# OliBomby/CM3P

Measured on AMD Instinct MI355X. Metric: contrastive training steps/sec (global beatmap-metadata pairs/sec), higher is better.
Workload: dtype bf16; 1 GPU; c2: default CM3P config, beatmap seq=4096, metadata seq=256, batch 32/GPU; global_batch=32, beatmap_seq=4096, metadata_seq=256, parallelism=dp1, weights=random init (reference init rules), fp32 master / bf16 GEMM operands

## Files before the change

### cm3p_amd/_lib.py

```python
from __future__ import annotations

import ctypes
import os
from ctypes import c_float, c_int, c_int64, c_uint64, c_void_p

import torch

F32, BF16 = 0, 1
ADD_A_BF16 = 16
POOL_PACKED = 2
GEMM_F32_TILED = 2
EPI_BF16, EPI_F32, EPI_F32_RESID, EPI_F32_BIAS, EPI_BF16_RESID = 0, 1, 2, 5, 7
ABI_VERSION = 20

_HERE = os.path.dirname(os.path.abspath(__file__))
LIB_PATH = os.environ.get("CM3P_HIP_LIB") or os.path.join(_HERE, "csrc", "libcm3p_hip.so")

_P, _I, _L, _F, _U64 = c_void_p, c_int, c_int64, c_float, c_uint64
_RETURNS_INT64 = {"cm3p_attn_bwd_fused_workspace_bytes", "cm3p_token_order_workspace_ints"}

SIGNATURES = {
    "cm3p_abi_version": [],
    "cm3p_layernorm_fwd": [_P, _I, _P, _P, _P, _P, _P, _L, _I, _F, _P],
    "cm3p_layernorm_bwd_blocks": [_L],
    "cm3p_layernorm_bwd": [_P, _I, _P, _I, _P, _P, _P, _P, _I, _P, _P, _P, _P, _L, _I, _P],
    "cm3p_embed_ln_fwd": [_P, _P, _I, _P, _P, _I, _P, _P, _P, _P, _P, _L, _I, _F, _L, _P],
    "cm3p_embed_ln_bwd": [_P, _I, _P, _P, _I, _P, _P, _I, _P, _P, _P, _P, _P, _P, _P, _L, _I, _L, _L, _P],
    "cm3p_embed_ln_bwd_sorted_chunk": [],
    "cm3p_embed_ln_bwd_sorted": [_P, _I, _P, _P, _P, _P, _I, _P, _P, _I, _P, _P, _P, _P, _P, _P, _P, _P, _P, _L, _I, _L, _L, _P],
    "cm3p_token_order_workspace_ints": [_L, _L],
    "cm3p_token_order": [_P, _L, _L, _P, _P, _P, _P],
    "cm3p_audio_slots": [_P, _L, _L, _P, _P, _P],
    "cm3p_gemm_bf16": [_P, _P, _P, _P, _L, _L, _L, _L, _L, _L, _I, _I, _I, _I, _P, _P],
    "cm3p_qkv_gemm_rope": [_P, _P, _P, _L, _L, _L, _P, _P, _I, _I, _I, _F, _P],
    "cm3p_gemm_wgrad_splits": [_L, _L, _L],
    "cm3p_gemm_route": [_L, _L, _L, _L, _L, _I, _I, _I, _I, _I, _I],
    "cm3p_gemm8p_set_grid": [_I],
    "cm3p_gemm8p_get_grid": [],
    "cm3p_build_ablation_flags": [],
    "cm3p_debug_set_dma_audit": [_P],
    "cm3p_cast_f32_bf16": [_P, _P, _L, _P],
    "cm3p_cast_f32_bf16_t": [_P, _P, _P, _L, _L, _P],
    "cm3p_cast_f32_bf16_t_multi": [_P, _I, _L, _P],
    "cm3p_add_f32": [_P, _P, _I, _P, _P, _L, _P],
    "cm3p_rope_table": [_P, _L, _P, _I, _P, _P, _P],
    "cm3p_rope_apply": [_P, _P, _P, _I, _I, _I, _L, _I, _P],
    "cm3p_attn_fwd": [_P, _P, _P, _P, _I, _I, _I, _I, _F, _I, _P],
    "cm3p_attn_fwd_impl": [_I, _I, _I, _I],
    "cm3p_attn_probs": [_P, _P, _P, _P, _I, _I, _I, _I, _F, _I, _P],
    "cm3p_attn_generic_supported": [_I],
    "cm3p_attn_fwd_generic": [_P, _P, _P, _P, _I, _I, _I, _I, _I, _F, _P],
    "cm3p_attn_bwd_generic": [_P, _P, _P, _P, _P, _P, _P, _I, _I, _I, _I, _I, _F, _P],
    "cm3p_attn_fwd_generic_dropout": [_P, _P, _P, _P, _I, _I, _I, _I, _I, _F, _I, _I, _U64, _P],
    "cm3p_attn_bwd_generic_dropout": [_P, _P, _P, _P, _P, _P, _P, _I, _I, _I, _I, _I, _F, _I, _I, _U64, _P],
    "cm3p_rope_apply_generic": [_P, _P, _P, _I, _I, _I, _I, _L, _I, _P],
    "cm3p_attn_bwd": [_P, _P, _P, _P, _P, _P, _P, _I, _I, _I, _I, _F, _P, _P, _L, _I, _I, _P],
    "cm3p_geglu_fwd": [_P, _P, _L, _I, _P],
    "cm3p_gemm_geglu": [_P, _P, _P, _L, _L, _L, _P],
    "cm3p_geglu_bwd": [_P, _P, _P, _L, _I, _P],
    "cm3p_dropout_f32": [_P, _P, _P, _P, _L, _I, _I, _P, _I, _I, _I, _I, _U64, _P],
    "cm3p_attn_fwd_dropout": [_P, _P, _P, _P, _I, _I, _I, _I, _F, _I, _I, _I, _U64, _P],
    "cm3p_attn_bwd_dropout": [_P, _P, _P, _P, _P, _P, _P, _I, _I, _I, _I, _F, _P, _P, _L, _I, _I, _I, _I, _U64, _P],
    "cm3p_attn_fwd_dropout_varlen": [_P, _P, _P, _P, _I, _I, _L, _I, _I, _F, _I, _I, _I, _U64, _P],
    "cm3p_attn_bwd_dropout_varlen": [_P, _P, _P, _P, _P, _P, _P, _I, _I, _L, _I, _I, _F, _P, _P, _I, _I, _I, _I, _U64, _P],
    "cm3p_geglu_fwd_dropout": [_P, _P, _L, _I, _I, _P, _I, _I, _I, _U64, _P],
    "cm3p_geglu_bwd_dropout": [_P, _P, _P, _L, _I, _I, _P, _I, _I, _I, _U64, _P],
    "cm3p_dropout_keep": [_P, _I, _I, _I, _I, _I, _I, _U64, _P],
    "cm3p_philox4x32_10_host": [_P, _P, _P, _L],
    "cm3p_gelu_fwd": [_P, _P, _L, _P],
    "cm3p_gelu_bwd": [_P, _P, _P, _L, _P],
    "cm3p_im2col_k3": [_P, _I, _P, _I, _I, _I, _I, _I, _P],
    "cm3p_col2im_k3": [_P, _P, _I, _I, _I, _I, _I, _P],
    "cm3p_bias_gelu_fwd": [_P, _P, _P, _P, _L, _I, _P],
    "cm3p_bias_gelu_bwd_blocks": [_L],
    "cm3p_bias_gelu_bwd": [_P, _I, _P, _P, _P, _P, _P, _L, _I, _P],
    "cm3p_pool_chunks": [_I],
    "cm3p_pool_fwd": [_P, _I, _P, _P, _P, _P, _I, _I, _I, _I, _P],
    "cm3p_pool_bwd": [_P, _P, _P, _P, _I, _I, _I, _I, _I, _P],
    "cm3p_gemm_f32": [_P, _P, _P, _I, _I, _I, _L, _L, _L, _L, _L, _F, _I, _P],
    "cm3p_l2norm_fwd": [_P, _P, _P, _I, _I, _P],
    "cm3p_l2norm_bwd": [_P, _P, _P, _P, _I, _I, _P],
    "cm3p_cross_entropy": [_P, _I, _I, _L, _L, _P, _P, _F, _P, _P, _P],
    "cm3p_cross_entropy_masked": [_P, _L, _I, _L, _P, _L, _F, _P, _P, _P, _P],
    "cm3p_inv_valid_count": [_P, _L, _L, _P, _P],
    "cm3p_ce_masked_stats": [_P, _L, _I, _L, _P, _L, _P, _P, _P],
    "cm3p_ce_masked_dlogits_blocks": [_L],
    "cm3p_ce_masked_dlogits_bf16": [_P, _L, _I, _L, _P, _L, _P, _P, _P, _P, _P, _P, _P],
    "cm3p_add_bias_f32": [_P, _P, _L, _I, _P],
    "cm3p_colsum_blocks": [_L],
    "cm3p_colsum_f32": [_P, _P, _P, _L, _I, _P],
    "cm3p_first_zero_index": [_P, _I, _I, _P, _P],
    "cm3p_scale_exp": [_P, _P, _P, _L, _P],
    "cm3p_scale_by": [_P, _P, _P, _L, _P],
    "cm3p_dot_f32": [_P, _P, _P, _L, _P],
    "cm3p_sum_f32": [_P, _P, _L, _F, _I, _P],
# ... 158 lines not shown
```

### cm3p_amd/csrc/common.h

```cpp
#pragma once
#include <hip/hip_runtime.h>
#include <stdint.h>

#include <atomic>
#include <initializer_list>
#include <mutex>
#include <type_traits>

#include "../../include/cm3p_hip.h"

typedef __attribute__((ext_vector_type(8))) __bf16 bf16x8;
typedef __attribute__((ext_vector_type(4))) __bf16 bf16x4;
typedef __attribute__((ext_vector_type(2))) __bf16 bf16x2;
typedef __attribute__((ext_vector_type(4))) float f32x4;
typedef __attribute__((ext_vector_type(8))) float f32x8;
typedef __attribute__((ext_vector_type(16))) float f32x16;

#define CM3P_WAVE 64
#define CM3P_EPI_BF16_ROPE 3
#define CM3P_EPI_BF16_AXPBY 4
#define CM3P_EPI_BF16_GEGLU 6

struct BatchArgs {
    int64_t a_stride = 0, b_stride = 0, c_stride = 0, r_stride = 0;
    const uint16_t* Rb = nullptr;
    float alpha = 1.f, beta = 0.f;
};

#ifndef CM3P_NT
#define CM3P_NT 7
#endif
typedef __attribute__((ext_vector_type(4))) uint32_t cm3p_u32x4;
typedef __attribute__((ext_vector_type(2))) uint32_t cm3p_u32x2;
template <bool NT>
__device__ __forceinline__ void gstore16(void* p, cm3p_u32x4 v) {
    if constexpr (NT) __builtin_nontemporal_store(v, static_cast<cm3p_u32x4*>(p));
    else *static_cast<cm3p_u32x4*>(p) = v;
}
template <bool NT>
__device__ __forceinline__ void gstore16(void* p, uint4 v) { gstore16<NT>(p, cm3p_u32x4{v.x, v.y, v.z, v.w}); }
template <bool NT>
__device__ __forceinline__ void gstore16f(void* p, __attribute__((ext_vector_type(4))) float v) {
    gstore16<NT>(p, __builtin_bit_cast(cm3p_u32x4, v));
}
template <bool NT>
__device__ __forceinline__ void gstore8(void* p, uint2 v) {
    if constexpr (NT) __builtin_nontemporal_store(cm3p_u32x2{v.x, v.y}, static_cast<cm3p_u32x2*>(p));
    else *static_cast<uint2*>(p) = v;
}
template <bool NT>
__device__ __forceinline__ uint4 gload16(const void* p) {
    if constexpr (NT) {
        const cm3p_u32x4 v = __builtin_nontemporal_load(static_cast<const cm3p_u32x4*>(p));
        return uint4{v[0], v[1], v[2], v[3]};
    } else {
        return *static_cast<const uint4*>(p);
    }
}

template <bool NT>
__device__ __forceinline__ uint2 gload8(const void* p) {
    if constexpr (NT) {
        const cm3p_u32x2 v = __builtin_nontemporal_load(static_cast<const cm3p_u32x2*>(p));
        return uint2{v[0], v[1]};
    } else {
        return *static_cast<const uint2*>(p);
    }
}
template <bool NT>
__device__ __forceinline__ __attribute__((ext_vector_type(4))) float gload16f(const void* p) {
    typedef __attribute__((ext_vector_type(4))) float f4;
    if constexpr (NT) return __builtin_nontemporal_load(static_cast<const f4*>(p));
    else return *static_cast<const f4*>(p);
}

#ifndef CM3P_DMA_AUDIT
#define CM3P_DMA_AUDIT 0
#endif
enum { CM3P_AUD_A = 0, CM3P_AUD_B = 1, CM3P_AUD_T0 = 2, CM3P_AUD_T1 = 3, CM3P_AUD_S0 = 4, CM3P_AUD_S1 = 5, CM3P_AUD_SLOTS = 8 };
#if CM3P_DMA_AUDIT
static __device__ unsigned long long* cm3p_audit_buf = nullptr;
static inline int cm3p_audit_set_local(void* buf) {
    return hipMemcpyToSymbol(HIP_SYMBOL(cm3p_audit_buf), &buf, sizeof(buf)) == hipSuccess ? CM3P_OK : CM3P_ERR_LAUNCH;
}
__device__ __forceinline__ void cm3p_audit(int id, const void* first_byte, int bytes) {
    unsigned long long* buf = cm3p_audit_buf;
    if (!buf) return;
    unsigned long long lo = (unsigned long long)(uintptr_t)first_byte, hi = lo + (unsigned long long)bytes - 1ull;
#pragma unroll
    for (int o = 32; o > 0; o >>= 1) {
        const unsigned long long l2 = __shfl_xor(lo, o, 64), h2 = __shfl_xor(hi, o, 64);
        lo = l2 < lo ? l2 : lo;
        hi = h2 > hi ? h2 : hi;
    }
    if ((threadIdx.x & 63) == 0) {
        atomicMin(buf + 2 * id, lo);
        atomicMax(buf + 2 * id + 1, hi);
    }
}
#define CM3P_AUDIT(id, addr, bytes) cm3p_audit((id), (addr), (bytes))
#else
#define CM3P_AUDIT(id, addr, bytes) ((void)0)
#endif

#define CM3P_LAUNCH_CHECK()                                         \
    do {                                                            \
        hipError_t e__ = hipGetLastError();                         \
        if (e__ != hipSuccess) return CM3P_ERR_LAUNCH;              \
    } while (0)
// ... 15 lines not shown
    if (cu[d] == 0) {
        hipDeviceProp_t prop;
        cu[d] = (hipGetDeviceProperties(&prop, d) == hipSuccess && prop.multiProcessorCount > 0) ? prop.multiProcessorCount : 256;
    }
    return cu[d];
}
struct Cm3pDevOnce {
    std::atomic<unsigned char> done[kCm3pMaxDevices] = {};
    std::mutex mu;
    template <class F>
    int run(F&& body) {
        int d = 0;
        const bool tracked = hipGetDevice(&d) == hipSuccess && d >= 0 && d < kCm3pMaxDevices;
        if (tracked && done[d].load(std::memory_order_acquire)) return CM3P_OK;
        std::lock_guard<std::mutex> g(mu);
        if (tracked && done[d].load(std::memory_order_relaxed)) return CM3P_OK;
        const int rc = body();
        if (rc == CM3P_OK && tracked) done[d].store(1, std::memory_order_release);
        return rc;
    }
};

static inline int cm3p_set_max_lds(std::initializer_list<const void*> kernels, int bytes) {
    for (const void* k : kernels)
        if (hipFuncSetAttribute(k, hipFuncAttributeMaxDynamicSharedMemorySize, bytes) != hipSuccess) return CM3P_ERR_LAUNCH;
    return CM3P_OK;
}

static inline bool cm3p_aligned16(const void* p) { return (reinterpret_cast<uintptr_t>(p) & 15u) == 0; }

__device__ __forceinline__ float bf16_bits_to_f32(uint16_t b) { return __builtin_bit_cast(float, (uint32_t)b << 16); }
__device__ __forceinline__ uint16_t f32_to_bf16_bits(float f) { return __builtin_bit_cast(uint16_t, (__bf16)f); }

typedef __attribute__((ext_vector_type(2))) float f32x2;
__device__ __forceinline__ f32x2 gelu_q_poly(f32x2 t) {
    f32x2 q = t * 0.24651730060577393f + (-1.1861149072647095f);
    q = q * t + 2.147474527359009f;
    q = q * t + (-1.6377531290054321f);
    q = q * t + 0.40232157707214355f;
    q = q * t + (-0.2687568664550781f);
    q = q * t + 0.1396300494670868f;
    q = q * t + 0.5397006273269653f;
    q = q * t + 1.4427292346954346f;
    q = q * t + (-1.8257482051849365f);
    return q;
}
__device__ __forceinline__ f32x2 gelu_t(f32x2 x) {
    const f32x2 ax = {__builtin_fabsf(x.x), __builtin_fabsf(x.y)};
    const f32x2 w = ax * 0.35355339059327373f + 1.0f;
    return f32x2{__builtin_amdgcn_rcpf(w.x), __builtin_amdgcn_rcpf(w.y)};
}
__device__ __forceinline__ void gelu_cdf_pdf2(f32x2 x, f32x2& cdf, f32x2& pdf) {
    const f32x2 t = gelu_t(x);
    const f32x2 q = gelu_q_poly(t);
    const f32x2 u = x * x * (-0.72134752044448170f);
    const f32x2 eu = {__builtin_amdgcn_exp2f(u.x), __builtin_amdgcn_exp2f(u.y)};
    const f32x2 eq = {__builtin_amdgcn_exp2f(q.x), __builtin_amdgcn_exp2f(q.y)};
    const f32x2 h = t * eu * eq * 0.5f;
    cdf.x = x.x < 0.f ? h.x : 1.0f - h.x;
    cdf.y = x.y < 0.f ? h.y : 1.0f - h.y;
    pdf = eu * 0.39894228040143267794f;
}
__device__ __forceinline__ f32x2 gelu_erf2(f32x2 x) {
    const f32x2 t = gelu_t(x);
    const f32x2 e = x * x * (-0.72134752044448170f) + gelu_q_poly(t);
    const f32x2 h = t * f32x2{__builtin_amdgcn_exp2f(e.x), __builtin_amdgcn_exp2f(e.y)} * 0.5f;
    const f32x2 cdf = {x.x < 0.f ? h.x : 1.0f - h.x, x.y < 0.f ? h.y : 1.0f - h.y};
    return x * cdf;
}
__device__ __forceinline__ f32x2 gelu_erf_grad2(f32x2 x) {
    f32x2 cdf, pdf;
    gelu_cdf_pdf2(x, cdf, pdf);
    return x * pdf + cdf;
}

__device__ __forceinline__ uint32_t pack_bf16x2(float lo, float hi) {
    bf16x2 v = {(__bf16)lo, (__bf16)hi};
    return __builtin_bit_cast(uint32_t, v);
}
__device__ __forceinline__ float bf16lo(uint32_t w) { return __builtin_bit_cast(float, w << 16); }
__device__ __forceinline__ float bf16hi(uint32_t w) { return __builtin_bit_cast(float, w & 0xffff0000u); }
__device__ __forceinline__ uint32_t add_bf16x2(uint32_t a, uint32_t b) { return pack_bf16x2(bf16lo(a) + bf16lo(b), bf16hi(a) + bf16hi(b)); }

struct RopeArgs {
    const float* cos;
    const float* sin;
    int S;
    int per_batch;
    int ncols;
    int q_cols = 0;
    float q_scale = 1.f;
};

enum { CM3P_GEMM_128 = 0, CM3P_GEMM_256 = 1, CM3P_GEMM_RING = 2 };
struct GemmRoute {
    int kernel;
    bool rebal;
    int splits;
    int64_t kchunk;
};
struct GemmCall {
    const void* A;
    const void* B;
    void* C;
    const float* R;
    int64_t M, N, K, lda, ldb, ldc;
    int a_kc, b_kc, epi;
    int64_t c_split_stride = 0;
    RopeArgs rope = RopeArgs{};
    BatchArgs bt = BatchArgs{};
    int batch = 0;
};
template <class F>
int cm3p_with_flag(bool v, F&& f) {
    return v ? f(std::true_type{}) : f(std::false_type{});
}
template <class F>
int cm3p_with_layout(bool a_kc, bool b_kc, F&& f) {
    return cm3p_with_flag(a_kc, [&](auto ak) { return cm3p_with_flag(b_kc, [&](auto bk) { return f(ak, bk); }); });
}
template <class F>
int cm3p_with_epilogue(int epi, F&& f) {
    switch (epi) {
        case CM3P_EPI_BF16: return f(std::integral_constant<int, CM3P_EPI_BF16>{});
        case CM3P_EPI_F32: return f(std::integral_constant<int, CM3P_EPI_F32>{});
        case CM3P_EPI_F32_RESID: return f(std::integral_constant<int, CM3P_EPI_F32_RESID>{});
        case CM3P_EPI_BF16_ROPE: return f(std::integral_constant<int, CM3P_EPI_BF16_ROPE>{});
        case CM3P_EPI_BF16_AXPBY: return f(std::integral_constant<int, CM3P_EPI_BF16_AXPBY>{});
        case CM3P_EPI_F32_BIAS: return f(std::integral_constant<int, CM3P_EPI_F32_BIAS>{});
        case CM3P_EPI_BF16_GEGLU: return f(std::integral_constant<int, CM3P_EPI_BF16_GEGLU>{});
        case CM3P_EPI_BF16_RESID: return f(std::integral_constant<int, CM3P_EPI_BF16_RESID>{});
        default: return CM3P_ERR_INTERNAL;
    }
}
constexpr bool cm3p_gemm_pair_exists(bool a_kc, bool b_kc, int epi) {
    return (epi != CM3P_EPI_BF16_ROPE && epi != CM3P_EPI_F32_BIAS && epi != CM3P_EPI_BF16_GEGLU) || (a_kc && b_kc);
}

template <bool INVERSE>
__device__ __forceinline__ void rope_rotate4(f32x4& a, f32x4& b, const float* cos_row, const float* sin_row, int d) {
    const f32x4 cs = *reinterpret_cast<const f32x4*>(cos_row + d);
    const f32x4 sn = *reinterpret_cast<const f32x4*>(sin_row + d);
    const f32x4 a0 = a, b0 = b;
    if constexpr (!INVERSE) {
        a = a0 * cs - b0 * sn;
        b = b0 * cs + a0 * sn;
    } else {
        a = a0 * cs + b0 * sn;
        b = b0 * cs - a0 * sn;
    }
}

__device__ __forceinline__ float wave_sum(float v) {
#pragma unroll
    for (int o = 32; o > 0; o >>= 1) v += __shfl_xor(v, o, 64);
    return v;
}
__device__ __forceinline__ float wave_max(float v) {
#pragma unroll
    for (int o = 32; o > 0; o >>= 1) v = fmaxf(v, __shfl_xor(v, o, 64));
    return v;
}

__device__ __forceinline__ bf16x4 lds_read_tr16(const void* p) {
    return __builtin_amdgcn_ds_read_tr16_b64_v4bf16((__attribute__((address_space(3))) bf16x4*)(p));
}

__device__ __forceinline__ bf16x8 cat_bf16x4(bf16x4 a, bf16x4 b) {
    return __builtin_shufflevector(a, b, 0, 1, 2, 3, 4, 5, 6, 7);
}
```

### cm3p_amd/csrc/elementwise.hip

```cpp
#include "common.h"
#include "dropout_rng.h"

namespace {

inline int ew_grid(int64_t items, int per_block = 256) {
    int64_t blocks = (items + per_block - 1) / per_block;
    if (blocks > 2048) blocks = 2048;
    if (blocks < 1) blocks = 1;
    return (int)blocks;
}

__device__ __forceinline__ void unpack8(const uint4 w, float (&f)[8]) {
    f[0] = bf16lo(w.x); f[1] = bf16hi(w.x); f[2] = bf16lo(w.y); f[3] = bf16hi(w.y);
    f[4] = bf16lo(w.z); f[5] = bf16hi(w.z); f[6] = bf16lo(w.w); f[7] = bf16hi(w.w);
}
__device__ __forceinline__ uint4 pack8(const float (&f)[8]) {
    return uint4{pack_bf16x2(f[0], f[1]), pack_bf16x2(f[2], f[3]), pack_bf16x2(f[4], f[5]), pack_bf16x2(f[6], f[7])};
}

__global__ __launch_bounds__(256) void cast_f32_bf16_kernel(const float* __restrict__ x, uint16_t* __restrict__ y, int64_t n4) {
    for (int64_t i = (int64_t)blockIdx.x * 256 + threadIdx.x; i < n4; i += (int64_t)gridDim.x * 256) {
        const f32x4 v = reinterpret_cast<const f32x4*>(x)[i];
        reinterpret_cast<uint2*>(y)[i] = uint2{pack_bf16x2(v.x, v.y), pack_bf16x2(v.z, v.w)};
    }
}

__global__ __launch_bounds__(256) void cast_f32_bf16_t_kernel(const float* __restrict__ x, uint16_t* __restrict__ y, uint16_t* __restrict__ yt,
                                                              int rows, int cols, int tiles_c) {
    __shared__ uint16_t tile[64][66];
    const int r0 = (blockIdx.x / tiles_c) * 64, c0 = (blockIdx.x % tiles_c) * 64;
    const int tid = threadIdx.x;
#pragma unroll
    for (int it = 0; it < 4; ++it) {
        const int r = it * 16 + (tid >> 4), c = (tid & 15) * 4;
        if (r0 + r < rows && c0 + c < cols) {
            const f32x4 v = *reinterpret_cast<const f32x4*>(x + (int64_t)(r0 + r) * cols + c0 + c);
            const uint32_t lo = pack_bf16x2(v.x, v.y), hi = pack_bf16x2(v.z, v.w);
            *reinterpret_cast<uint2*>(y + (int64_t)(r0 + r) * cols + c0 + c) = uint2{lo, hi};
            tile[r][c] = (uint16_t)lo;
            tile[r][c + 1] = (uint16_t)(lo >> 16);
            tile[r][c + 2] = (uint16_t)hi;
            tile[r][c + 3] = (uint16_t)(hi >> 16);
        }
    }
    __syncthreads();
#pragma unroll
    for (int it = 0; it < 2; ++it) {
        const int c = it * 32 + (tid >> 3), r = (tid & 7) * 8;
        if (c0 + c < cols && r0 + r < rows) {
            uint32_t w[4];
#pragma unroll
            for (int k = 0; k < 4; ++k) w[k] = (uint32_t)tile[r + 2 * k][c] | ((uint32_t)tile[r + 2 * k + 1][c] << 16);
            *reinterpret_cast<uint4*>(yt + (int64_t)(c0 + c) * rows + r0 + r) = uint4{w[0], w[1], w[2], w[3]};
        }
    }
}

__global__ __launch_bounds__(256) void cast_f32_bf16_t_multi_kernel(const int64_t* __restrict__ table, int n) {
    __shared__ uint16_t tile[64][66];
    int lo = 0, hi = n - 1;
    while (lo < hi) {
        const int mid = (lo + hi + 1) >> 1;
        if (table[6 * mid + 5] <= (int64_t)blockIdx.x) lo = mid;
        else hi = mid - 1;
    }
    const float* x = reinterpret_cast<const float*>(table[6 * lo]);
    uint16_t* y = reinterpret_cast<uint16_t*>(table[6 * lo + 1]);
    uint16_t* yt = reinterpret_cast<uint16_t*>(table[6 * lo + 2]);
    const int rows = (int)table[6 * lo + 3], cols = (int)table[6 * lo + 4];
    const int blk = (int)((int64_t)blockIdx.x - table[6 * lo + 5]);
    const int tiles_c = (cols + 63) / 64;
    const int r0 = (blk / tiles_c) * 64, c0 = (blk % tiles_c) * 64;
    const int tid = threadIdx.x;
#pragma unroll
    for (int it = 0; it < 4; ++it) {
        const int r = it * 16 + (tid >> 4), c = (tid & 15) * 4;
        if (r0 + r < rows && c0 + c < cols) {
            const f32x4 v = *reinterpret_cast<const f32x4*>(x + (int64_t)(r0 + r) * cols + c0 + c);
            const uint32_t lo2 = pack_bf16x2(v.x, v.y), hi2 = pack_bf16x2(v.z, v.w);
            *reinterpret_cast<uint2*>(y + (int64_t)(r0 + r) * cols + c0 + c) = uint2{lo2, hi2};
            tile[r][c] = (uint16_t)lo2;
            tile[r][c + 1] = (uint16_t)(lo2 >> 16);
            tile[r][c + 2] = (uint16_t)hi2;
            tile[r][c + 3] = (uint16_t)(hi2 >> 16);
        }
    }
    __syncthreads();
#pragma unroll
    for (int it = 0; it < 2; ++it) {
        const int c = it * 32 + (tid >> 3), r = (tid & 7) * 8;
        if (c0 + c < cols && r0 + r < rows) {
            uint32_t w[4];
#pragma unroll
            for (int k = 0; k < 4; ++k) w[k] = (uint32_t)tile[r + 2 * k][c] | ((uint32_t)tile[r + 2 * k + 1][c] << 16);
            *reinterpret_cast<uint4*>(yt + (int64_t)(c0 + c) * rows + r0 + r) = uint4{w[0], w[1], w[2], w[3]};
        }
    }
}

template <bool B_BF16>
__global__ __launch_bounds__(256) void add_f32_kernel(const float* __restrict__ a, const void* __restrict__ b, float* y32,
                                                      uint16_t* __restrict__ y16, int64_t n4) {
    for (int64_t i = (int64_t)blockIdx.x * 256 + threadIdx.x; i < n4; i += (int64_t)gridDim.x * 256) {
        f32x4 v = reinterpret_cast<const f32x4*>(a)[i];
        if constexpr (B_BF16) {
            const uint2 w = reinterpret_cast<const uint2*>(b)[i];
            v += f32x4{bf16lo(w.x), bf16hi(w.x), bf16lo(w.y), bf16hi(w.y)};
        } else {
            v += reinterpret_cast<const f32x4*>(b)[i];
        }
        if (y32) reinterpret_cast<f32x4*>(y32)[i] = v;
        if (y16) reinterpret_cast<uint2*>(y16)[i] = uint2{pack_bf16x2(v.x, v.y), pack_bf16x2(v.z, v.w)};
    }
}

template <bool B_BF16>
__global__ __launch_bounds__(256) void add_bf16_kernel(const uint16_t* a, const void* __restrict__ b, uint16_t* y, int64_t n4) {
    for (int64_t i = (int64_t)blockIdx.x * 256 + threadIdx.x; i < n4; i += (int64_t)gridDim.x * 256) {
        const uint2 wa = reinterpret_cast<const uint2*>(a)[i];
        f32x4 v = f32x4{bf16lo(wa.x), bf16hi(wa.x), bf16lo(wa.y), bf16hi(wa.y)};
        if constexpr (B_BF16) {
            const uint2 w = reinterpret_cast<const uint2*>(b)[i];
            v += f32x4{bf16lo(w.x), bf16hi(w.x), bf16lo(w.y), bf16hi(w.y)};
        } else {
            v += reinterpret_cast<const f32x4*>(b)[i];
        }
        reinterpret_cast<uint2*>(y)[i] = uint2{pack_bf16x2(v.x, v.y), pack_bf16x2(v.z, v.w)};
    }
}

__global__ __launch_bounds__(256) void rope_table_kernel(const int64_t* __restrict__ pos, const float* __restrict__ inv_freq,
                                                         float* __restrict__ cos_out, float* __restrict__ sin_out, int64_t n,
                                                         int half) {
    for (int64_t i = (int64_t)blockIdx.x * 256 + threadIdx.x; i < n * half; i += (int64_t)gridDim.x * 256) {
        const int64_t p = i / half;
        const int j = (int)(i % half);
        const float ang = (float)pos[p] * inv_freq[j];
        cos_out[i] = cosf(ang);
        sin_out[i] = sinf(ang);
    }
}

template <bool INVERSE>
__global__ __launch_bounds__(256) void rope_apply_kernel(uint16_t* __restrict__ qkv, const float* __restrict__ cos_tab,
                                                         const float* __restrict__ sin_tab, int64_t T, int S, int nh,
                                                         int64_t pos_batch_stride) {
    const int64_t per_tok = (int64_t)2 * nh * 4;
    const int64_t total = T * per_tok;
    for (int64_t i = (int64_t)blockIdx.x * 256 + threadIdx.x; i < total; i += (int64_t)gridDim.x * 256) {
        const int64_t t = i / per_tok;
        const int r = (int)(i % per_tok);
        const int part = r / (nh * 4);
        const int h = (r / 4) % nh;
        const int c = r & 3;
        const int64_t b = t / S, s = t % S;
        const int64_t prow = (pos_batch_stride ? b * pos_batch_stride : 0) + s;
        uint16_t* base = qkv + (t * 3 + part) * (int64_t)nh * 64 + h * 64 + c * 8;
        float x1[8], x2[8], cs[8], sn[8];
        unpack8(*reinterpret_cast<const uint4*>(base), x1);
        unpack8(*reinterpret_cast<const uint4*>(base + 32), x2);
        const f32x4* cp = reinterpret_cast<const f32x4*>(cos_tab + prow * 32 + c * 8);
        const f32x4* sp = reinterpret_cast<const f32x4*>(sin_tab + prow * 32 + c * 8);
        const f32x4 c0 = cp[0], c1 = cp[1], s0 = sp[0], s1 = sp[1];
// ... 3 lines not shown
#pragma unroll
        for (int j = 0; j < 8; ++j) {
            if constexpr (!INVERSE) {
                y1[j] = x1[j] * cs[j] - x2[j] * sn[j];
                y2[j] = x2[j] * cs[j] + x1[j] * sn[j];
            } else {
                y1[j] = x1[j] * cs[j] + x2[j] * sn[j];
                y2[j] = x2[j] * cs[j] - x1[j] * sn[j];
            }
        }
        *reinterpret_cast<uint4*>(base) = pack8(y1);
        *reinterpret_cast<uint4*>(base + 32) = pack8(y2);
    }
}

#ifndef CM3P_GEGLU_X2
#define CM3P_GEGLU_X2 3
#endif
template <int NI>
struct GegluWalk {
    int64_t dq, t0;
    int dr, c0, c8;
    __device__ __forceinline__ GegluWalk(int I) {
        c8 = I / 8;
        const int64_t stride = (int64_t)gridDim.x * 256 * NI, first = ((int64_t)blockIdx.x * 4 + (threadIdx.x >> 6)) * (64 * NI) + (threadIdx.x & 63);
        dq = stride / c8;
        dr = (int)(stride % c8);
        t0 = first / c8;
        c0 = (int)(first % c8);
    }
    __device__ __forceinline__ bool next(int64_t T, int64_t (&tt)[NI], int (&cc)[NI], bool (&ok)[NI]) {
        if (t0 >= T) return false;
        if (c0 >= c8) {
            c0 -= c8;
            if (++t0 >= T) return false;
        }
        tt[0] = t0, cc[0] = c0, ok[0] = true;
#pragma unroll
        for (int k = 1; k < NI; ++k) {
            tt[k] = tt[k - 1];
            cc[k] = cc[k - 1] + 64;
            while (cc[k] >= c8) {
                cc[k] -= c8;
                ++tt[k];
            }
            ok[k] = tt[k] < T;
            if (!ok[k]) tt[k] = t0, cc[k] = c0;
        }
        t0 += dq;
        c0 += dr;
        return true;
    }
};

__global__ __launch_bounds__(256) void geglu_fwd_kernel(const uint16_t* __restrict__ h, uint16_t* __restrict__ g, int64_t T, int I) {
    constexpr int NI = CM3P_GEGLU_X2 + 1;
    GegluWalk<NI> walk(I);
    int64_t tt[NI];
    int cc[NI];
    bool ok[NI];
    while (walk.next(T, tt, cc, ok)) {
        uint4 ha[NI], hb[NI];
#pragma unroll
        for (int k = 0; k < NI; ++k) {
            ha[k] = gload16<(CM3P_NT & 128) != 0>(h + tt[k] * 2 * I + cc[k] * 8);
            hb[k] = gload16<(CM3P_NT & 128) != 0>(h + tt[k] * 2 * I + I + cc[k] * 8);
        }
#pragma unroll
        for (int k = 0; k < NI; ++k) {
            float a[8], b[8], y[8];
            unpack8(ha[k], a);
            unpack8(hb[k], b);
#pragma unroll
            for (int j = 0; j < 8; j += 2) {
                const f32x2 gl = gelu_erf2(f32x2{a[j], a[j + 1]});
                y[j] = gl.x * b[j];
                y[j + 1] = gl.y * b[j + 1];
            }
            if (ok[k]) gstore16<(CM3P_NT & 16) != 0>(g + tt[k] * I + cc[k] * 8, pack8(y));
        }
    }
}

__device__ __forceinline__ void geglu_bwd_item_f(const uint4 ha, const uint4 hb, const float (&d)[8], uint4& oa, uint4& ob) {
    float a[8], b[8], da[8], db[8];
    unpack8(ha, a);
    unpack8(hb, b);
#pragma unroll
    for (int j = 0; j < 8; j += 2) {
        const f32x2 av = {a[j], a[j + 1]};
        f32x2 cdf, pdf;
        gelu_cdf_pdf2(av, cdf, pdf);
        const f32x2 gr = av * pdf + cdf, gl = av * cdf;
        da[j] = d[j] * b[j] * gr.x;
        da[j + 1] = d[j + 1] * b[j + 1] * gr.y;
        db[j] = d[j] * gl.x;
        db[j + 1] = d[j + 1] * gl.y;
    }
    oa = pack8(da);
    ob = pack8(db);
}

__device__ __forceinline__ void geglu_bwd_item(const uint4 ha, const uint4 hb, const uint4 hd, uint4& oa, uint4& ob) {
    float d[8];
    unpack8(hd, d);
    geglu_bwd_item_f(ha, hb, d, oa, ob);
}

__global__ __launch_bounds__(256) void geglu_bwd_kernel(const uint16_t* __restrict__ dg, const uint16_t* __restrict__ h,
                                                        uint16_t* __restrict__ dh, int64_t T, int I) {
    constexpr int NI = CM3P_GEGLU_X2 + 1;
    GegluWalk<NI> walk(I);
    int64_t tt[NI];
    int cc[NI];
    bool ok[NI];
    while (walk.next(T, tt, cc, ok)) {
        uint4 ha[NI], hb[NI], hd[NI];
#pragma unroll
        for (int k = 0; k < NI; ++k) {
            ha[k] = gload16<(CM3P_NT & 128) != 0>(h + tt[k] * 2 * I + cc[k] * 8);
            hb[k] = gload16<(CM3P_NT & 128) != 0>(h + tt[k] * 2 * I + I + cc[k] * 8);
            hd[k] = gload16<(CM3P_NT & 128) != 0>(dg + tt[k] * I + cc[k] * 8);
        }
#pragma unroll
        for (int k = 0; k < NI; ++k) {
            uint4 oa, ob;
            geglu_bwd_item(ha[k], hb[k], hd[k], oa, ob);
            if (ok[k]) {
                gstore16<(CM3P_NT & 16) != 0>(dh + tt[k] * 2 * I + cc[k] * 8, oa);
                gstore16<(CM3P_NT & 16) != 0>(dh + tt[k] * 2 * I + I + cc[k] * 8, ob);
            }
        }
    }
}

struct DropArgs {
    uint64_t seed;
    uint32_t c3, thr;
    float scale;
    int S, nseq;
    const int* cu;
};

__device__ __forceinline__ uint32_t drop_keep8(const DropArgs& d, int64_t t, uint32_t f8) {
    uint32_t b, s;
    cm3p_drop::row_to_seq(t, d.S, d.cu, d.nseq, b, s);
    return cm3p_drop::keep8(d.seed, f8, s, b, d.c3, d.thr);
}

__global__ __launch_bounds__(256) void dropout_f32_kernel(const float* x, const float* resid, float* y32, uint16_t* __restrict__ y16, int64_t rows,
                                                          int H, DropArgs d) {
    const int h8 = H / 8;
    const int64_t n = rows * h8;
    for (int64_t i = (int64_t)blockIdx.x * 256 + threadIdx.x; i < n; i += (int64_t)gridDim.x * 256) {
        const int64_t t = i / h8;
        const uint32_t m = drop_keep8(d, t, (uint32_t)(i - t * h8));
        f32x4 v0 = reinterpret_cast<const f32x4*>(x)[2 * i], v1 = reinterpret_cast<const f32x4*>(x)[2 * i + 1];
#pragma unroll
        for (int j = 0; j < 4; ++j) {
            v0[j] = (m >> j) & 1u ? v0[j] * d.scale : 0.f;
            v1[j] = (m >> (4 + j)) & 1u ? v1[j] * d.scale : 0.f;
        }
        if (resid) {
            v0 += reinterpret_cast<const f32x4*>(resid)[2 * i];
            v1 += reinterpret_cast<const f32x4*>(resid)[2 * i + 1];
        }
        if (y32) {
            reinterpret_cast<f32x4*>(y32)[2 * i] = v0;
            reinterpret_cast<f32x4*>(y32)[2 * i + 1] = v1;
        }
        if (y16)
            reinterpret_cast<uint4*>(y16)[i] =
                uint4{pack_bf16x2(v0.x, v0.y), pack_bf16x2(v0.z, v0.w), pack_bf16x2(v1.x, v1.y), pack_bf16x2(v1.z, v1.w)};
    }
}

__global__ __launch_bounds__(256) void geglu_drop_fwd_kernel(const uint16_t* __restrict__ h, uint16_t* __restrict__ g, int64_t T, int I,
                                                             DropArgs d) {
    const int i8 = I / 8;
    const int64_t n = T * i8;
    for (int64_t i = (int64_t)blockIdx.x * 256 + threadIdx.x; i < n; i += (int64_t)gridDim.x * 256) {
        const int64_t t = i / i8;
        const int c = (int)(i - t * i8);
        const uint32_t m = drop_keep8(d, t, (uint32_t)c);
        float a[8], b[8], y[8];
// ... 505 lines not shown
```

### cm3p_amd/csrc/gemm.hip

```cpp
#include <stdlib.h>

#include "common.h"

namespace {

constexpr int BM = 128, BN = 128, BK = 64;
constexpr int kStageBytes = BM * BK * 2;

__device__ __forceinline__ int kc_off(int r, int c) { return r * 128 + ((c ^ (r & 7)) << 4); }
__device__ __forceinline__ int ks_off(int k, int idx) {
    const int f = (k & 3) | (((k >> 3) & 1) << 2);
    return k * 256 + ((((idx >> 4) ^ f) & 7) << 5) + ((idx & 15) << 1);
}

template <bool KC>
struct TileLoader {
    const uint16_t* ptr[4];
    bool row_ok[4];
    int koff[4];
    int lds[4];
    int64_t kstep;

    __device__ __forceinline__ void init(const uint16_t* base, int64_t ld, int64_t idx0, int64_t extent, int64_t kbeg, int tid) {
#pragma unroll
// ... 90 lines not shown
        const char* sb = sa + kStageBytes;
        const bool more = kt + 1 < nk;
        if (more) {
            la.load(ra, kbeg + (int64_t)(kt + 1) * BK, kend);
            lb.load(rb, kbeg + (int64_t)(kt + 1) * BK, kend);
        }
#pragma unroll
        for (int kk = 0; kk < 2; ++kk) {
            bf16x8 fa[4], fb[4];
#pragma unroll
            for (int i = 0; i < 4; ++i) fa[i] = load_frag<A_KC>(sa, wm * 64 + i * 16, kk, lane);
#pragma unroll
            for (int j = 0; j < 4; ++j) fb[j] = load_frag<B_KC>(sb, wn * 64 + j * 16, kk, lane);
#pragma unroll
            for (int i = 0; i < 4; ++i)
#pragma unroll
                for (int j = 0; j < 4; ++j)
                    acc[i][j] = __builtin_amdgcn_mfma_f32_16x16x32_bf16(fb[j], fa[i], acc[i][j], 0, 0, 0);
        }
        if (more) {
            char* na = smem + ((kt + 1) & 1) * 2 * kStageBytes;
            la.store(na, ra);
            lb.store(na + kStageBytes, rb);
        }
        __syncthreads();
    }

#pragma unroll
    for (int i = 0; i < 4; ++i) {
        const int64_t m = m0 + wm * 64 + i * 16 + (lane & 15);
        if (m >= M) continue;
        if constexpr (EPI == CM3P_EPI_BF16_ROPE) {
            if (n0 + wn * 64 < rope.ncols) {
                const int64_t prow = rope.per_batch ? m : m % rope.S;
#pragma unroll
                for (int j = 0; j < 2; ++j)
                    rope_rotate4<false>(acc[i][j], acc[i][j + 2], rope.cos + prow * 32, rope.sin + prow * 32, j * 16 + 4 * (lane >> 4));
                if (n0 + wn * 64 < rope.q_cols) {
#pragma unroll
                    for (int j = 0; j < 4; ++j) acc[i][j] *= rope.q_scale;
                }
            }
        }
#pragma unroll
        for (int j = 0; j < 4; ++j) {
            const int64_t n = n0 + wn * 64 + j * 16 + 4 * (lane >> 4);
            if (n >= N) continue;
            f32x4 v = acc[i][j];
            if constexpr (EPI == CM3P_EPI_BF16 || EPI == CM3P_EPI_BF16_ROPE) {
                uint16_t* C = static_cast<uint16_t*>(Cv);
                *reinterpret_cast<uint2*>(C + m * ldc + n) = uint2{pack_bf16x2(v.x, v.y), pack_bf16x2(v.z, v.w)};
            } else if constexpr (EPI == CM3P_EPI_BF16_RESID) {
                uint16_t* C = static_cast<uint16_t*>(Cv);
                const uint2 r = *reinterpret_cast<const uint2*>(reinterpret_cast<const uint16_t*>(R) + m * ldc + n);
                *reinterpret_cast<uint2*>(C + m * ldc + n) = uint2{add_bf16x2(pack_bf16x2(v.x, v.y), r.x), add_bf16x2(pack_bf16x2(v.z, v.w), r.y)};
            } else if constexpr (EPI == CM3P_EPI_BF16_AXPBY) {
                uint16_t* C = static_cast<uint16_t*>(Cv) + (int64_t)blockIdx.y * bt.c_stride;
                v *= bt.alpha;
                if (bt.Rb) {
                    const uint2 r = *reinterpret_cast<const uint2*>(bt.Rb + (int64_t)blockIdx.y * bt.r_stride + m * ldc + n);
                    v += bt.beta * f32x4{bf16lo(r.x), bf16hi(r.x), bf16lo(r.y), bf16hi(r.y)};
                }
                *reinterpret_cast<uint2*>(C + m * ldc + n) = uint2{pack_bf16x2(v.x, v.y), pack_bf16x2(v.z, v.w)};
            } else {
                float* C = static_cast<float*>(Cv) + (int64_t)blockIdx.z * c_split_stride;
                if constexpr (EPI == CM3P_EPI_F32_RESID) v += *reinterpret_cast<const f32x4*>(R + m * ldc + n);
                if constexpr (EPI == CM3P_EPI_F32_BIAS) v += *reinterpret_cast<const f32x4*>(R + n);
                *reinterpret_cast<f32x4*>(C + m * ldc + n) = v;
            }
        }
    }
}

__global__ __launch_bounds__(256) void splitk_reduce_kernel(const float* __restrict__ ws, float* __restrict__ out, int64_t n4,
                                                            int splits, int64_t stride4) {
    for (int64_t i = (int64_t)blockIdx.x * 256 + threadIdx.x; i < n4; i += (int64_t)gridDim.x * 256) {
        f32x4 s = reinterpret_cast<const f32x4*>(ws)[i];
        for (int z = 1; z < splits; ++z) s += reinterpret_cast<const f32x4*>(ws)[i + z * stride4];
        reinterpret_cast<f32x4*>(out)[i] = s;
    }
}

template <bool A_KC, bool B_KC, int EPI>
constexpr bool has_instance = cm3p_gemm_pair_exists(A_KC, B_KC, EPI) && EPI != CM3P_EPI_BF16_GEGLU;

int launch128(const GemmRoute& r, const GemmCall& g, hipStream_t s) {
    const int tiles_m = (int)((g.M + BM - 1) / BM), tiles_n = (int)((g.N + BN - 1) / BN);
    const dim3 grid(tiles_m * tiles_n, g.batch > 0 ? g.batch : 1, r.splits);
    const size_t lds = 4 * kStageBytes;
    const uint16_t* a = static_cast<const uint16_t*>(g.A);
    const uint16_t* b = static_cast<const uint16_t*>(g.B);
    return cm3p_with_layout(g.a_kc, g.b_kc, [&](auto ak, auto bk) {
        return cm3p_with_epilogue(g.epi, [&](auto e) {
            constexpr bool AK = decltype(ak)::value, BK = decltype(bk)::value;
            constexpr int E = decltype(e)::value;
            if constexpr (has_instance<AK, BK, E>) {
                gemm_bf16_kernel<AK, BK, E><<<grid, 256, lds, s>>>(a, b, g.C, g.R, g.M, g.N, g.K, g.lda, g.ldb, g.ldc, tiles_n, r.kchunk,
                                                                 g.c_split_stride, g.rope, g.bt);
                return CM3P_OK;
            } else {
                return CM3P_ERR_INTERNAL;
            }
        });
    });
}

}

int cm3p_gemm256_dispatch(const GemmRoute& r, const GemmCall& g, hipStream_t s);
int cm3p_gemm8p_dispatch(const GemmRoute& r, const GemmCall& g, hipStream_t s);

static inline int64_t tiles_of(int64_t M, int64_t N, int t) { return ((M + t - 1) / t) * ((N + t - 1) / t); }
constexpr int64_t kBigItems = 200, kBigBatchItems = 128;

static GemmRoute cm3p_gemm_route_of(int64_t M, int64_t N, int64_t K, int64_t lda, int64_t ldb, bool a_kc, bool b_kc, int epi,
                                    int split_k, int rope_cols, int batch) {
    GemmRoute r{CM3P_GEMM_128, false, 1, K};
    const bool batched = epi == CM3P_EPI_BF16_AXPBY;
    if (M <= 0 || N <= 0 || K <= 0 || split_k < 1 || epi < 0 || epi > CM3P_EPI_BF16_RESID || batched != (batch > 0) ||
        !cm3p_gemm_pair_exists(a_kc, b_kc, epi)) {
        r.kernel = CM3P_ERR_INVALID;
        return r;
    }
    const char* impl = getenv("CM3P_GEMM_IMPL");
    const bool no_ring = impl && impl[0] == '2', small_only = impl && impl[0] == '1';
    static const bool no_rebal = [] { const char* e = getenv("CM3P_G8P_REBAL"); return e && e[0] == '0'; }();
    if (split_k > 1) {
        const int64_t q = (K % 128 == 0) ? 128 : 64;
        r.kchunk = ((K + split_k - 1) / split_k + q - 1) / q * q;
        r.splits = (int)((K + r.kchunk - 1) / r.kchunk);
    }
    const int64_t items = tiles_of(M, N, 256) * (batched ? batch : r.splits);
    const bool ring_ok = M % 8 == 0 && N % 8 == 0 && lda * 16 < (int64_t(1) << 31) && ldb * 16 < (int64_t(1) << 31);
    bool big = K % 64 == 0 && r.kchunk % 64 == 0 && items >= (batched ? kBigBatchItems : kBigItems);
    if (epi == CM3P_EPI_BF16_GEGLU) {
        if (!(big && N % 64 == 0 && ring_ok)) r.kernel = CM3P_ERR_INVALID;
        else r.kernel = no_ring ? CM3P_GEMM_256 : CM3P_GEMM_RING;
    } else if (batched) {
        const bool filled = M * N * batch * 10 >= items * 65536 * 7;
        big = big && filled && (a_kc || !b_kc) && ring_ok && !no_ring;
        if (big) r.kernel = CM3P_GEMM_RING;
    } else {
        big = big && !small_only;
        if (epi == CM3P_EPI_BF16_ROPE) big = big && rope_cols % 256 == 0 && M < (int64_t(1) << 31);
        if (big) r.kernel = (ring_ok && !no_ring) ? CM3P_GEMM_RING : CM3P_GEMM_256;
    }
    if (r.kernel > CM3P_GEMM_128) {
        const int64_t last = K - (int64_t)(r.splits - 1) * r.kchunk;
        r.rebal = !no_rebal && (r.kchunk / 64) % 2 == 0 && (last / 64) % 2 == 0;
    }
    return r;
}

static int run_routed(const GemmRoute& r, const GemmCall& g, hipStream_t s) {
    int rc = CM3P_ERR_INVALID;
    if (r.kernel == CM3P_GEMM_RING) rc = cm3p_gemm8p_dispatch(r, g, s);
    else if (r.kernel == CM3P_GEMM_256) rc = cm3p_gemm256_dispatch(r, g, s);
    else if (r.kernel == CM3P_GEMM_128) rc = launch128(r, g, s);
    if (rc != CM3P_OK) return rc;
    CM3P_LAUNCH_CHECK();
    return CM3P_OK;
}

int cm3p_ablation_flags_attention();
int cm3p_ablation_flags_attention_bwd_fused();
int cm3p_ablation_flags_gemm256();
int cm3p_ablation_flags_gemm8p();
int cm3p_ablation_flags_attention_fwd();
#if CM3P_DMA_AUDIT
int cm3p_audit_set_attention_fwd(void*);
int cm3p_audit_set_gemm8p(void*);
int cm3p_audit_set_gemm256(void*);
int cm3p_audit_set_attention(void*);
int cm3p_audit_set_attention_bwd_fused(void*);
#endif

extern "C" {

int cm3p_build_ablation_flags(void) {
    return (cm3p_ablation_flags_attention() != 0) | (cm3p_ablation_flags_attention_bwd_fused() != 0) << 2 |
           (cm3p_ablation_flags_gemm256() != 0) << 3 | (cm3p_ablation_flags_gemm8p() != 0) << 4 | (CM3P_DMA_AUDIT != 0) << 5 |
           (cm3p_ablation_flags_attention_fwd() != 0) << 6;
}

int cm3p_debug_set_dma_audit(void* buf) {
#if CM3P_DMA_AUDIT
    int rc = cm3p_audit_set_gemm8p(buf);
    if (rc == CM3P_OK) rc = cm3p_audit_set_gemm256(buf);
    if (rc == CM3P_OK) rc = cm3p_audit_set_attention(buf);
    if (rc == CM3P_OK) rc = cm3p_audit_set_attention_bwd_fused(buf);
    if (rc == CM3P_OK) rc = cm3p_audit_set_attention_fwd(buf);
    return rc;
#else
    (void)buf;
    return CM3P_ERR_INVALID;
#endif
}

int cm3p_gemm_wgrad_splits(int64_t M, int64_t N, int64_t K) {
    const int64_t t256 = tiles_of(M, N, 256);
    if (K % 64 == 0 && K >= 8192) {
        int64_t s = 256 / t256;
        if (s > K / 2048) s = K / 2048;
        if (s < 1) s = 1;
        if (t256 * s >= kBigItems) return (int)s;
    }
    const int64_t t128 = tiles_of(M, N, 128);
    if (t128 >= 512 || K <= 1024) return 1;
    int64_t s = (1024 + t128 - 1) / t128;
    if (s > K / 512) s = K / 512;
    return (int)(s < 1 ? 1 : s);
}

int cm3p_gemm_route(int64_t M, int64_t N, int64_t K, int64_t lda, int64_t ldb, int a_kc, int b_kc, int epilogue, int split_k,
                    int rope_cols, int batch) {
    const GemmRoute r = cm3p_gemm_route_of(M, N, K, lda, ldb, a_kc != 0, b_kc != 0, epilogue, split_k, rope_cols, batch);
    return r.kernel < 0 ? CM3P_ERR_INVALID : (r.kernel | (r.rebal ? 4 : 0) | r.splits << 3);
}

int cm3p_qkv_gemm_rope(const void* x, const void* Wqkv, void* qkv, int64_t M, int64_t N, int64_t K, const float* cos_tab,
                       const float* sin_tab, int S, int per_batch, int rope_cols, float q_scale, void* stream) {
    CM3P_REQUIRE(x && Wqkv && qkv && cos_tab && sin_tab && M > 0 && N > 0 && K > 0 && S > 0);
    CM3P_REQUIRE(cm3p_aligned16(x) && cm3p_aligned16(Wqkv) && cm3p_aligned16(qkv) && cm3p_aligned16(cos_tab) && cm3p_aligned16(sin_tab));
    CM3P_REQUIRE(K % 8 == 0 && N % 64 == 0 && rope_cols % 64 == 0 && rope_cols >= 0 && rope_cols <= N);
    CM3P_REQUIRE(per_batch || M % S == 0);
    CM3P_REQUIRE(q_scale > 0.f && rope_cols % 2 == 0);
    const GemmRoute r = cm3p_gemm_route_of(M, N, K, K, K, true, true, CM3P_EPI_BF16_ROPE, 1, rope_cols, 0);
    CM3P_REQUIRE(r.kernel >= 0);
    GemmCall g{x, Wqkv, qkv, nullptr, M, N, K, K, K, N, 1, 1, CM3P_EPI_BF16_ROPE};
    g.rope = RopeArgs{cos_tab, sin_tab, S, per_batch, rope_cols, rope_cols / 2, q_scale};
    return run_routed(r, g, static_cast<hipStream_t>(stream));
}

int cm3p_gemm_bf16(const void* A, const void* B, void* C, const float* R, int64_t M, int64_t N, int64_t K, int64_t lda,
                   int64_t ldb, int64_t ldc, int a_kc, int b_kc, int epilogue, int split_k, float* workspace, void* stream) {
    CM3P_REQUIRE(A && B && C && M > 0 && N > 0 && K > 0);
    CM3P_REQUIRE((epilogue >= CM3P_EPI_BF16 && epilogue <= CM3P_EPI_F32_RESID) || epilogue == CM3P_EPI_F32_BIAS || epilogue == CM3P_EPI_BF16_RESID);
    CM3P_REQUIRE(cm3p_aligned16(A) && cm3p_aligned16(B) && cm3p_aligned16(C));
    CM3P_REQUIRE(lda % 8 == 0 && ldb % 8 == 0 && ldc % 4 == 0 && N % 4 == 0);
    CM3P_REQUIRE(a_kc ? (K % 8 == 0 && lda >= K) : (M % 8 == 0 && lda >= M));
    CM3P_REQUIRE(b_kc ? (K % 8 == 0 && ldb >= K) : (N % 8 == 0 && ldb >= N));
    CM3P_REQUIRE(ldc >= N);
    CM3P_REQUIRE((epilogue != CM3P_EPI_F32_RESID && epilogue != CM3P_EPI_F32_BIAS && epilogue != CM3P_EPI_BF16_RESID) || (R && cm3p_aligned16(R)));
    CM3P_REQUIRE(epilogue != CM3P_EPI_BF16_RESID || (N % 8 == 0 && ldc % 8 == 0));
    CM3P_REQUIRE(split_k >= 1 && (split_k == 1 || (epilogue == CM3P_EPI_F32 && workspace && cm3p_aligned16(workspace) && ldc == N)));
    const GemmRoute r = cm3p_gemm_route_of(M, N, K, lda, ldb, a_kc != 0, b_kc != 0, epilogue, split_k, 0, 0);
    CM3P_REQUIRE(r.kernel >= 0);
    hipStream_t s = static_cast<hipStream_t>(stream);
    GemmCall g{A, B, C, R, M, N, K, lda, ldb, ldc, a_kc != 0, b_kc != 0, epilogue};
    if (r.splits > 1) {
        g.C = workspace;
        g.c_split_stride = M * N;
    }
    const int rc = run_routed(r, g, s);
    if (rc != CM3P_OK) return rc;
    if (r.splits > 1) {
        const int64_t n4 = M * N / 4;
        int64_t blocks = (n4 + 255) / 256;
        if (blocks > 2048) blocks = 2048;
        splitk_reduce_kernel<<<(int)blocks, 256, 0, s>>>(workspace, static_cast<float*>(C), n4, r.splits, n4);
        CM3P_LAUNCH_CHECK();
    }
    return CM3P_OK;
}

int cm3p_gemm_geglu(const void* x, const void* w_interleaved, void* a, int64_t T, int64_t I, int64_t K, void* stream) {
    CM3P_REQUIRE(x && w_interleaved && a && T > 0 && I > 0 && K > 0);
    CM3P_REQUIRE(cm3p_aligned16(x) && cm3p_aligned16(w_interleaved) && cm3p_aligned16(a));
    GemmRoute r = cm3p_gemm_route_of(T, 2 * I, K, K, K, true, true, CM3P_EPI_BF16_GEGLU, 1, 0, 0);
    CM3P_REQUIRE(r.kernel >= 0);
    r.kernel = CM3P_GEMM_RING;
    const GemmCall g{x, w_interleaved, a, nullptr, T, 2 * I, K, K, K, I, 1, 1, CM3P_EPI_BF16_GEGLU};
    return run_routed(r, g, static_cast<hipStream_t>(stream));
}

int cm3p_gemm_bf16_batched(const void* A, const void* B, void* C, const void* R, int batch, int64_t M, int64_t N, int64_t K,
                           int64_t lda, int64_t ldb, int64_t ldc, int64_t stride_a, int64_t stride_b, int64_t stride_c,
                           int64_t stride_r, int a_kc, int b_kc, float alpha, float beta, void* stream) {
    CM3P_REQUIRE(A && B && C && batch > 0 && batch <= 65535 && M > 0 && N > 0 && K > 0);
    CM3P_REQUIRE(cm3p_aligned16(A) && cm3p_aligned16(B) && cm3p_aligned16(C) && (!R || cm3p_aligned16(R)));
    CM3P_REQUIRE(lda % 8 == 0 && ldb % 8 == 0 && ldc % 8 == 0 && N % 8 == 0 && ldc >= N);
    CM3P_REQUIRE(stride_a % 8 == 0 && stride_b % 8 == 0 && stride_c % 8 == 0 && stride_r % 8 == 0);
    CM3P_REQUIRE(a_kc ? (K % 8 == 0 && lda >= K) : (M % 8 == 0 && lda >= M));
    CM3P_REQUIRE(b_kc ? (K % 8 == 0 && ldb >= K) : (N % 8 == 0 && ldb >= N));
    const GemmRoute r = cm3p_gemm_route_of(M, N, K, lda, ldb, a_kc != 0, b_kc != 0, CM3P_EPI_BF16_AXPBY, 1, 0, batch);
    CM3P_REQUIRE(r.kernel >= 0);
    GemmCall g{A, B, C, nullptr, M, N, K, lda, ldb, ldc, a_kc != 0, b_kc != 0, CM3P_EPI_BF16_AXPBY};
    g.bt = BatchArgs{stride_a, stride_b, stride_c, stride_r, static_cast<const uint16_t*>(R), alpha, beta};
    g.batch = batch;
    return run_routed(r, g, static_cast<hipStream_t>(stream));
}

}
```

### cm3p_amd/csrc/gemm256.hip

```cpp
#include "common.h"

namespace {

constexpr int TM = 256, TN = 256, TK = 64;
#ifndef CM3P_G256_WN
#define CM3P_G256_WN 4
#endif
constexpr int kWN = CM3P_G256_WN;
constexpr int kThreads = 128 * kWN;
constexpr int kNJ = 16 / kWN;
constexpr int kWaveN = TN / kWN;
#ifndef CM3P_G256_ABL
#define CM3P_G256_ABL 0
#endif
constexpr int kPieces = 16 / kWN;
constexpr int kItems = 2048 / kThreads;
constexpr int kOperandBytes = TM * TK * 2;
constexpr int kStage = 2 * kOperandBytes;

__device__ __forceinline__ int kc_off(int r, int c) { return r * 128 + ((c ^ (r & 7)) << 4); }
__device__ __forceinline__ int ksf(int k) { return (k & 3) | (((k >> 3) & 1) << 2); }
__device__ __forceinline__ int ks_off(int k, int idx) { return k * 512 + (((idx >> 4) ^ ksf(k)) << 5) + ((idx & 15) << 1); }

__device__ __forceinline__ void glds16(const void* gsrc, char* lds_wave_base) {
// ... 250 lines not shown
                        if (m < M && n < N) {
                            uint4 x = *reinterpret_cast<const uint4*>(ebuf + r * kRow + ch * 16);
                            if constexpr (EPI == CM3P_EPI_BF16_RESID) {
                                const uint4 rb = *reinterpret_cast<const uint4*>(reinterpret_cast<const uint16_t*>(R) + m * ldc + n);
                                x = uint4{add_bf16x2(x.x, rb.x), add_bf16x2(x.y, rb.y), add_bf16x2(x.z, rb.z), add_bf16x2(x.w, rb.w)};
                            }
                            if constexpr (EPI == CM3P_EPI_BF16) {
                                if (n + 8 > N) {
                                    *reinterpret_cast<uint2*>(C + m * ldc + n) = uint2{x.x, x.y};
                                    continue;
                                }
                            }
                            *reinterpret_cast<uint4*>(C + m * ldc + n) = x;
                        }
                    }
                }
                lds_barrier();
            }
        } else {
            constexpr int kRow = TN * 4 + 16;
            float* C = static_cast<float*>(Cv) + (int64_t)z * c_split_stride;
            f32x4 rres[kItems];
            auto load_resid = [&](int pass) {
                if constexpr (EPI == CM3P_EPI_F32_RESID) {
#pragma unroll
                    for (int u = 0; u < kItems; ++u) {
                        const int id = tid + kThreads * u, r = id >> 6, ch = id & 63;
                        const int64_t m = m0 + pass * 32 + r, n = n0 + ch * 4;
                        rres[u] = (m < M && n < N) ? *reinterpret_cast<const f32x4*>(R + m * ldc + n) : f32x4{0.f, 0.f, 0.f, 0.f};
                    }
                }
                if constexpr (EPI == CM3P_EPI_F32_BIAS) {
                    if (pass == 0) {
#pragma unroll
                        for (int u = 0; u < kItems; ++u) {
                            const int64_t n = n0 + ((tid + kThreads * u) & 63) * 4;
                            rres[u] = n < N ? *reinterpret_cast<const f32x4*>(R + n) : f32x4{0.f, 0.f, 0.f, 0.f};
                        }
                    }
                }
            };
            load_resid(0);
#pragma unroll
            for (int pass = 0; pass < 8; ++pass) {
                if (wm == (pass >> 2)) {
#pragma unroll
                    for (int i2 = 0; i2 < 2; ++i2)
#pragma unroll
                        for (int j = 0; j < kNJ; ++j) {
                            const f32x4 a = acc[(pass & 3) * 2 + i2][j];
                            const int r = i2 * 16 + (lane & 15), cidx = wn * kWaveN + j * 16 + 4 * (lane >> 4);
                            *reinterpret_cast<f32x4*>(ebuf + r * kRow + cidx * 4) = a;
                        }
                }
                lds_barrier();
                f32x4 rcur[kItems];
#pragma unroll
                for (int u = 0; u < kItems; ++u) rcur[u] = rres[u];
                if (pass < 7) load_resid(pass + 1);
#pragma unroll
                for (int u = 0; u < kItems; ++u) {
                    const int id = tid + kThreads * u, r = id >> 6, ch = id & 63;
                    const int64_t m = m0 + pass * 32 + r, n = n0 + ch * 4;
                    if (m < M && n < N) {
                        f32x4 a = *reinterpret_cast<const f32x4*>(ebuf + r * kRow + ch * 16);
                        if constexpr (EPI == CM3P_EPI_F32_RESID || EPI == CM3P_EPI_F32_BIAS) a += rcur[u];
                        *reinterpret_cast<f32x4*>(C + m * ldc + n) = a;
                    }
                }
                lds_barrier();
            }
        }

        if (!has_next) break;
        v = vn;
        m0 = m0n;
        n0 = n0n;
        z = zn;
        nk = nkn;
    }
}

template <bool A_KC, bool B_KC, int EPI>
constexpr bool has_instance = cm3p_gemm_pair_exists(A_KC, B_KC, EPI) && EPI != CM3P_EPI_BF16_GEGLU && EPI != CM3P_EPI_BF16_AXPBY;

}

int cm3p_gemm256_dispatch(const GemmRoute& r, const GemmCall& g, hipStream_t s) {
    const int tiles_m = (int)((g.M + TM - 1) / TM), tiles_n = (int)((g.N + TN - 1) / TN);
    const int ntiles = tiles_m * tiles_n, total = ntiles * r.splits;
    const int num_cu = cm3p_num_cu();
    const dim3 grid(total < num_cu ? total : num_cu);
    const size_t lds = 2 * kStage;
    const uint16_t* a = static_cast<const uint16_t*>(g.A);
    const uint16_t* b = static_cast<const uint16_t*>(g.B);
    return cm3p_with_layout(g.a_kc, g.b_kc, [&](auto ak, auto bk) {
        return cm3p_with_epilogue(g.epi, [&](auto e) {
            constexpr bool AK = decltype(ak)::value, BK = decltype(bk)::value;
            constexpr int E = decltype(e)::value;
            if constexpr (has_instance<AK, BK, E>) {
                static Cm3pDevOnce once;
                const int rc_once = once.run([&] { return cm3p_set_max_lds({(const void*)gemm256_kernel<AK, BK, E>}, (int)lds); });
                if (rc_once != CM3P_OK) return rc_once;
                gemm256_kernel<AK, BK, E><<<grid, kThreads, lds, s>>>(a, b, g.C, g.R, g.M, g.N, g.K, g.lda, g.ldb, g.ldc, tiles_n, ntiles, total,
                                                                    r.kchunk, g.c_split_stride, g.rope);
                return CM3P_OK;
            } else {
                return CM3P_ERR_INTERNAL;
            }
        });
    });
}

int cm3p_ablation_flags_gemm256() { return (CM3P_G256_ABL) | ((CM3P_G256_WN != 4) << 8); }
#if CM3P_DMA_AUDIT
int cm3p_audit_set_gemm256(void* buf) { return cm3p_audit_set_local(buf); }
#endif
```

### cm3p_amd/csrc/gemm8p.hip

```cpp
#include <stdlib.h>

#include <type_traits>

#include "common.h"

#ifndef CM3P_G8P_ABL
#define CM3P_G8P_ABL 0
#endif
#ifndef CM3P_G8P_DELAY
#define CM3P_G8P_DELAY 10
#endif

namespace {

constexpr int kHalf = 16384;
constexpr int kRing = 8 * kHalf;
constexpr int kEpiWave = 4096;
constexpr int kLds8p = kRing + 8 * kEpiWave;
enum { kAL = 0, kAH = 1, kBL = 2, kBH = 3 };
__host__ __device__ constexpr int slot_off(int par, int kind) { return (par * 4 + kind) * kHalf; }

template <int IMM, int AUD = CM3P_AUD_A>
__device__ __forceinline__ void glds_s(uint32_t voff, const char* sbase, uint32_t ldsw) {
    CM3P_AUDIT(AUD, sbase + voff, 16);
// ... 306 lines not shown
                if constexpr (EPI == CM3P_EPI_BF16_RESID) {
                    const int r0 = lane >> 3, r1 = 8 + (lane >> 3), ch = lane & 7;
                    const bool col_ok = FULL || nw + ch * 8 < N;
                    res0 = (FULL || (col_ok && mw + i4 * 16 + r0 < M)) ? __builtin_bit_cast(u32x4, gload16<(CM3P_NT & 64) != 0>(Rb + (uint32_t)(i4 * 16 + r0) * ldcb + ch * 16))
                                                                       : u32x4{0u, 0u, 0u, 0u};
                    res1 = (FULL || (col_ok && mw + i4 * 16 + r1 < M)) ? __builtin_bit_cast(u32x4, gload16<(CM3P_NT & 64) != 0>(Rb + (uint32_t)(i4 * 16 + r1) * ldcb + ch * 16))
                                                                       : u32x4{0u, 0u, 0u, 0u};
                }
#pragma unroll
                for (int j4 = 0; j4 < 4; ++j4) {
                    const f32x4 a = acc[i4][j4];
                    const int row = lane & 15, s8 = (j4 * 4 + (lane >> 4)) ^ ((row & 7) << 1);
                    *reinterpret_cast<uint2*>(eb + row * 128 + s8 * 8) = uint2{pack_bf16x2(a.x, a.y), pack_bf16x2(a.z, a.w)};
                }
                G8P_LANE_XCHG_FENCE();
                if (rotate) {
                    const int row = lane >> 2, dc = lane & 3;
                    char* pa = eb + row * 128 + ((dc ^ (row & 7)) << 4);
                    char* pb = eb + row * 128 + (((dc + 4) ^ (row & 7)) << 4);
                    const u32x4 xa = *reinterpret_cast<const u32x4*>(pa);
                    const u32x4 xb = *reinterpret_cast<const u32x4*>(pb);
                    const f32x4 c0 = tc0, c1 = tc1, s0 = ts0, s1 = ts1;
                    if (i4 < 7) tab_load(i4 + 1, tc0, tc1, ts0, ts1);
                    {
                        const float cs[8] = {c0.x, c0.y, c0.z, c0.w, c1.x, c1.y, c1.z, c1.w};
                        const float sn[8] = {s0.x, s0.y, s0.z, s0.w, s1.x, s1.y, s1.z, s1.w};
                        u32x4 oa, ob;
#pragma unroll
                        for (int t = 0; t < 4; ++t) {
                            const float a0 = bf16lo(xa[t]), a1 = bf16hi(xa[t]), b0 = bf16lo(xb[t]), b1 = bf16hi(xb[t]);
                            oa[t] = pack_bf16x2(qs * (a0 * cs[2 * t] - b0 * sn[2 * t]), qs * (a1 * cs[2 * t + 1] - b1 * sn[2 * t + 1]));
                            ob[t] = pack_bf16x2(qs * (b0 * cs[2 * t] + a0 * sn[2 * t]), qs * (b1 * cs[2 * t + 1] + a1 * sn[2 * t + 1]));
                        }
                        *reinterpret_cast<u32x4*>(pa) = oa;
                        *reinterpret_cast<u32x4*>(pb) = ob;
                    }
                    G8P_LANE_XCHG_FENCE();
                }
                {
                    const int r0 = lane >> 3, r1 = 8 + (lane >> 3), ch = lane & 7;
                    u32x4 x0 = *reinterpret_cast<const u32x4*>(eb + r0 * 128 + ((ch ^ (r0 & 7)) << 4));
                    u32x4 x1 = *reinterpret_cast<const u32x4*>(eb + r1 * 128 + ((ch ^ (r1 & 7)) << 4));
                    G8P_LANE_XCHG_FENCE();
                    if constexpr (EPI == CM3P_EPI_BF16_RESID) {
#pragma unroll
                        for (int t = 0; t < 4; ++t) {
                            x0[t] = add_bf16x2(x0[t], res0[t]);
                            x1[t] = add_bf16x2(x1[t], res1[t]);
                        }
                    }
                    const bool col_ok = FULL || nw + ch * 8 < N;
                    if (FULL || (col_ok && mw + i4 * 16 + r0 < M)) G8P_GLOBAL(gstore16<(CM3P_NT & 1) != 0>(Cb + (uint32_t)(i4 * 16 + r0) * ldcb + ch * 16, x0));
                    if (FULL || (col_ok && mw + i4 * 16 + r1 < M)) G8P_GLOBAL(gstore16<(CM3P_NT & 1) != 0>(Cb + (uint32_t)(i4 * 16 + r1) * ldcb + ch * 16, x1));
                    if constexpr (CM3P_G8P_ABL & 1) asm volatile("" ::"v"(x0), "v"(x1));
                }
            }
        } else if constexpr (EPI == CM3P_EPI_BF16_GEGLU) {
            char* Cb = reinterpret_cast<char*>(static_cast<uint16_t*>(Cv) + mw * ldc + nw / 2);
            const uint32_t ldcb = (uint32_t)ldc * 2;
#pragma unroll
            for (int i4 = 0; i4 < 8; ++i4) {
                char* eb = ebuf + (i4 & 1) * 2048;
#pragma unroll
                for (int j4 = 0; j4 < 4; ++j4) {
                    const f32x4 a = acc[i4][j4];
                    const int row = lane & 15, s8 = (j4 * 4 + (lane >> 4)) ^ ((row & 7) << 1);
                    *reinterpret_cast<uint2*>(eb + row * 128 + s8 * 8) = uint2{pack_bf16x2(a.x, a.y), pack_bf16x2(a.z, a.w)};
                }
                G8P_LANE_XCHG_FENCE();
                const int row = lane >> 2, dc = lane & 3;
                const u32x4 xh = *reinterpret_cast<const u32x4*>(eb + row * 128 + ((dc ^ (row & 7)) << 4));
                const u32x4 xg = *reinterpret_cast<const u32x4*>(eb + row * 128 + (((dc + 4) ^ (row & 7)) << 4));
                G8P_LANE_XCHG_FENCE();
                u32x4 y;
#pragma unroll
                for (int t = 0; t < 4; ++t) {
                    const f32x2 gl = gelu_erf2(f32x2{bf16lo(xh[t]), bf16hi(xh[t])});
                    y[t] = pack_bf16x2(gl.x * bf16lo(xg[t]), gl.y * bf16hi(xg[t]));
                }
                if (FULL || (mw + i4 * 16 + row < M && nw + dc * 8 < N))
                    G8P_GLOBAL(gstore16<(CM3P_NT & 1) != 0>(Cb + (uint32_t)(i4 * 16 + row) * ldcb + dc * 16, y));
                if constexpr (CM3P_G8P_ABL & 1) asm volatile("" ::"v"(y));
            }
        } else if constexpr (EPI == CM3P_EPI_BF16_AXPBY) {
            char* Cb = reinterpret_cast<char*>(static_cast<uint16_t*>(Cv) + (int64_t)z * bt.c_stride + mw * ldc + nw);
            const char* Rb = reinterpret_cast<const char*>(bt.Rb + (int64_t)z * bt.r_stride + mw * ldc + nw);
            const uint32_t ldcb = (uint32_t)ldc * 2;
            const int lrow = lane >> 4, lch = lane & 15;
            const uint32_t loff = (uint32_t)lrow * ldcb + lch * 8;
            const bool col_ok = FULL || nw + lch * 4 < N;
#pragma unroll
            for (int i4 = 0; i4 < 8; ++i4) {
                uint2 r[4];
                if (bt.Rb) {
#pragma unroll
                    for (int u = 0; u < 4; ++u) {
                        const int row = i4 * 16 + u * 4;
                        r[u] = (FULL || (col_ok && mw + row + lrow < M)) ? *reinterpret_cast<const uint2*>(Rb + loff + (uint32_t)row * ldcb) : uint2{0u, 0u};
                    }
                }
#pragma unroll
                for (int j4 = 0; j4 < 4; ++j4) {
                    const int row = lane & 15, ch = j4 * 4 + (lane >> 4);
                    *reinterpret_cast<f32x4*>(ebuf + row * 256 + ((ch ^ row) << 4)) = acc[i4][j4];
                }
                G8P_LANE_XCHG_FENCE();
                f32x4 x[4];
#pragma unroll
                for (int u = 0; u < 4; ++u) {
                    const int row = u * 4 + lrow;
                    x[u] = *reinterpret_cast<const f32x4*>(ebuf + row * 256 + ((lch ^ row) << 4));
                }
                G8P_LANE_XCHG_FENCE();
#pragma unroll
                for (int u = 0; u < 4; ++u) {
                    f32x4 v = x[u];
                    v *= bt.alpha;
                    if (bt.Rb) v += bt.beta * f32x4{bf16lo(r[u].x), bf16hi(r[u].x), bf16lo(r[u].y), bf16hi(r[u].y)};
                    const int row = i4 * 16 + u * 4;
                    if (FULL || (col_ok && mw + row + lrow < M))
                        G8P_GLOBAL(*reinterpret_cast<uint2*>(Cb + loff + (uint32_t)row * ldcb) = (uint2{pack_bf16x2(v.x, v.y), pack_bf16x2(v.z, v.w)}));
                    if constexpr (CM3P_G8P_ABL & 1) asm volatile("" ::"v"(v));
                }
            }
        } else {
            char* Cb = reinterpret_cast<char*>(static_cast<float*>(Cv) + (int64_t)z * c_split_stride + mw * ldc + nw);
            const char* Rb = reinterpret_cast<const char*>(R + mw * ldc + nw);
            const uint32_t ldcb = (uint32_t)ldc * 4;
            const int lrow = lane >> 4, lch = lane & 15;
            const uint32_t loff = (uint32_t)lrow * ldcb + lch * 16;
            const bool col_ok = FULL || nw + lch * 4 < N;
            f32x4 rnext[4];
            auto load_r = [&](int i4) {
                if constexpr (EPI == CM3P_EPI_F32_RESID && !(CM3P_G8P_ABL & 1)) {
#pragma unroll
                    for (int u = 0; u < 4; ++u) {
                        const int row = i4 * 16 + u * 4;
                        rnext[u] = (FULL || (col_ok && mw + row + lrow < M)) ? gload16f<(CM3P_NT & 64) != 0>(Rb + loff + (uint32_t)row * ldcb)
                                                                             : f32x4{0.f, 0.f, 0.f, 0.f};
                    }
                }
            };
            f32x4 bias = f32x4{0.f, 0.f, 0.f, 0.f};
            if constexpr (EPI == CM3P_EPI_F32_BIAS) {
                if (col_ok) bias = *reinterpret_cast<const f32x4*>(R + nw + lch * 4);
            }
            load_r(0);
#pragma unroll
            for (int i4 = 0; i4 < 8; ++i4) {
#pragma unroll
                for (int j4 = 0; j4 < 4; ++j4) {
                    const int row = lane & 15, ch = j4 * 4 + (lane >> 4);
                    *reinterpret_cast<f32x4*>(ebuf + row * 256 + ((ch ^ row) << 4)) = acc[i4][j4];
                }
                G8P_LANE_XCHG_FENCE();
                f32x4 x[4];
#pragma unroll
                for (int u = 0; u < 4; ++u) {
                    const int row = u * 4 + lrow;
                    x[u] = *reinterpret_cast<const f32x4*>(ebuf + row * 256 + ((lch ^ row) << 4));
                }
                G8P_LANE_XCHG_FENCE();
#pragma unroll
                for (int u = 0; u < 4; ++u) {
                    if constexpr (EPI == CM3P_EPI_F32_RESID && !(CM3P_G8P_ABL & 1)) x[u] += rnext[u];
                    if constexpr (EPI == CM3P_EPI_F32_BIAS) x[u] += bias;
// ... 104 lines not shown
```

### cm3p_amd/encoder.py

```python
from __future__ import annotations

import os
import weakref
from typing import Optional

import torch
from torch import nn

from . import kernels as K

Tensor = torch.Tensor


def _check_supported(cfg):
    H, nh = cfg.hidden_size, cfg.num_attention_heads
    problems = []
    if H % nh or H // nh not in (16, 32, 64, 96, 128):
        problems.append(f"head_dim must be 64 (or 16 / 32 on the generic kernels, or 96 / 128 on the wide-head MFMA kernels); hidden_size={H}, heads={nh}")
    if getattr(cfg, "hidden_activation", "gelu") != "gelu":
        problems.append("hidden_activation must be 'gelu'")
    for flag in ("norm_bias", "attention_bias", "mlp_bias"):
        if getattr(cfg, flag, False):
            problems.append(f"{flag}=True is not supported (the reference configs never set it)")
    for p in ("attention_dropout", "embedding_dropout", "mlp_dropout"):
# ... 5 lines not shown
    if problems:
        raise NotImplementedError("cm3p_amd HIP encoder: " + "; ".join(problems))


class CM3PAttentionParams(nn.Module):
    def __init__(self, cfg):
        super().__init__()
        self.Wqkv = nn.Linear(cfg.hidden_size, 3 * cfg.hidden_size, bias=False)
        self.Wo = nn.Linear(cfg.hidden_size, cfg.hidden_size, bias=False)


class CM3PMLPParams(nn.Module):
    def __init__(self, cfg):
        super().__init__()
        self.Wi = nn.Linear(cfg.hidden_size, 2 * cfg.intermediate_size, bias=False)
        self.Wo = nn.Linear(cfg.intermediate_size, cfg.hidden_size, bias=False)


class CM3PEncoderLayerParams(nn.Module):
    def __init__(self, cfg, layer_idx: int):
        super().__init__()
        self.attn_norm = nn.Identity() if layer_idx == 0 else nn.LayerNorm(cfg.hidden_size, eps=cfg.norm_eps, bias=False)
        self.attn = CM3PAttentionParams(cfg)
        self.mlp_norm = nn.LayerNorm(cfg.hidden_size, eps=cfg.norm_eps, bias=False)
        self.mlp = CM3PMLPParams(cfg)


class CM3PEmbeddingParams(nn.Module):
    def __init__(self, cfg):
        super().__init__()
        self.tok_embeddings = nn.Embedding(cfg.vocab_size, cfg.hidden_size, padding_idx=getattr(cfg, "pad_token_id", None))
        self.norm = nn.LayerNorm(cfg.hidden_size, eps=cfg.norm_eps, bias=False)


def _f32(w: Tensor) -> Tensor:
    return w if w.dtype == torch.float32 else w.float()


def _bf16_weight(w: Tensor) -> Tensor:
    w = w.detach()
    if w.dtype == torch.bfloat16:
        return w
    if w.dtype != torch.float32:
        w = w.float()
    return K.cast_bf16(w.contiguous())


_eval_weights: dict = {}
K._other_caches.append(_eval_weights)


def invalidate_weight_cache() -> None:
    _eval_weights.clear()


def _bf16_weight_cached(w: Tensor, geglu_rows: bool = False) -> Tensor:
    key = (id(w), geglu_rows)
    hit = _eval_weights.get(key)
    if hit is not None and hit[0]() is w and hit[1] == w._version and hit[2] == w.data_ptr():
        return hit[3]
    wb = _bf16_weight(w)
    if geglu_rows:
        wb = wb.index_select(0, K.geglu_interleave_index(w.shape[0] // 2, wb.device)).contiguous()
    if wb.data_ptr() != w.data_ptr():
        if len(_eval_weights) > 4096:
            for k in [k for k, v in _eval_weights.items() if v[0]() is None]:
                del _eval_weights[k]
        _eval_weights[key] = (weakref.ref(w), w._version, w.data_ptr(), wb)
    return wb


def _bf16_weight_pair(w: Tensor, want_t: bool):
    if not want_t:
        return _bf16_weight_cached(w), None
    w = w.detach()
    if w.dtype == torch.float32 and w.dim() == 2 and w.shape[0] % 8 == 0 and w.shape[1] % 8 == 0:
        return K.cast_bf16_with_transpose(w.contiguous())
    return _bf16_weight(w), None


class _Geometry:

    __slots__ = ("B", "S", "H", "I", "nh", "L", "eps", "windows", "key_mask", "rope", "per_batch_pos", "save", "cu", "max_s", "checkpoint",
                 "handoff", "attn_out", "wcast", "hd", "drop", "bf16")


def _hand_upstream(geo: _Geometry, gx32: Tensor, gx16: Optional[Tensor]) -> None:
    geo.handoff = (gx32, gx16)


def _take_from_downstream(geo: _Geometry, dy: Tensor):
    h, geo.handoff = geo.handoff, None
    if h is not None and h[1] is not None and h[0].data_ptr() == dy.data_ptr() and h[0].shape == dy.shape and dy.dtype == torch.float32 \
            and dy.is_contiguous():
        return h[0], h[1]
    g = dy.float().contiguous()
    if g.data_ptr() == dy.data_ptr():
        g = g.clone()
    return g, K.cast_bf16(g)


def _take_bf16_from_downstream(geo: _Geometry, dy: Tensor) -> Tensor:
    h, geo.handoff = geo.handoff, None
    if h is not None and h[0].data_ptr() == dy.data_ptr() and h[0].shape == dy.shape and dy.dtype == torch.bfloat16 and dy.is_contiguous():
        return h[0]
    g = dy.to(torch.bfloat16).contiguous()
    if g.data_ptr() == dy.data_ptr():
        g = g.clone()
    return g


def _layer_forward(geo: _Geometry, i: int, x: Tensor, wb, want_stats: bool):
    w_an, Wqkv_b, Wo_b, w_mn, Wi_b, Wo2_b = wb[:6]
    B, S, nh = geo.B, geo.S, geo.nh
    scale = geo.hd ** -0.5
    cos, sin = geo.rope[i]
    ad = (geo.drop.attn, geo.drop.seed, i) if geo.drop is not None and geo.drop.attn else None
    if i == 0:
        xn, mean_a, rstd_a = (x if x.dtype == torch.bfloat16 else K.cast_bf16(x)), None, None
    else:
        _, xn, mean_a, rstd_a = K.layernorm_fwd(x, w_an, geo.eps, False, True, want_stats)
    if geo.hd != 64:
        qkv = K.linear_fwd(xn, Wqkv_b)
        K.rope_apply_generic_(qkv, cos, sin, B, S, nh, geo.hd, geo.per_batch_pos)
        o, lse = K.attn_fwd_generic(qkv, geo.key_mask, B, S, nh, geo.hd, geo.windows[i], scale, drop=ad)
    elif geo.cu is not None:
        qkv = K.qkv_linear_rope(xn, Wqkv_b, cos, sin, S, geo.per_batch_pos, q_scale=K.SOFTMAX_Q_SCALE)
        o, lse = K.attn_fwd_varlen(qkv, geo.cu, B, geo.max_s, nh, geo.windows[i], scale, prescaled=True, drop=ad)
    else:
        qkv = K.qkv_linear_rope(xn, Wqkv_b, cos, sin, S, geo.per_batch_pos, q_scale=K.SOFTMAX_Q_SCALE)
        o, lse = K.attn_fwd(qkv, geo.key_mask, B, S, nh, geo.windows[i], scale, prescaled=True, drop=ad)
        if geo.attn_out is not None and len(geo.attn_out) == i:
            geo.attn_out.append(K.attn_probs(qkv, lse, geo.key_mask, B, S, nh, geo.windows[i], scale, prescaled=True))
    if ad is not None:
        x_mid = K.dropout_f32(K.linear_fwd_f32(o, Wo_b), ad[0], ad[1], i, K.SITE_ATTN_OUT, geo.S, geo.cu, resid=x)
    else:
        x_mid = K.linear_fwd(o, Wo_b, resid=x)
    _, xn2, mean_m, rstd_m = K.layernorm_fwd(x_mid, w_mn, geo.eps, False, True, want_stats)
    if len(wb) > 6 and wb[6] is not None:
        h, g = None, K.gemm_geglu(xn2, wb[6])
    else:
        h = K.linear_fwd(xn2, Wi_b)
        if geo.drop is not None and geo.drop.mlp:
            g = K.geglu_fwd_dropout(h, geo.drop.mlp, geo.drop.seed, i, geo.S, geo.cu)
        else:
            g = K.geglu_fwd(h)
    x_out = K.linear_fwd(g, Wo2_b, resid=x_mid)
    return x_out, (x, xn, mean_a, rstd_a, qkv, o, lse, x_mid, xn2, mean_m, rstd_m, h, g)


def _attn_backward(geo: _Geometry, i: int, qkv: Tensor, o: Tensor, do: Tensor, lse: Tensor, ad: Optional[tuple]) -> Tensor:
    B, S, nh, window, scale = geo.B, geo.S, geo.nh, geo.windows[i], geo.hd ** -0.5
    if geo.hd != 64:
        dqkv = K.attn_bwd_generic(qkv, o, do, lse, geo.key_mask, B, S, nh, geo.hd, window, scale, drop=ad)
        return K.rope_apply_generic_(dqkv, geo.rope[i][0], geo.rope[i][1], B, S, nh, geo.hd, geo.per_batch_pos, inverse=True)
    if geo.cu is not None:
        return K.attn_bwd_varlen(qkv, o, do, lse, geo.cu, B, geo.max_s, nh, window, scale, geo.rope[i], prescaled=True, drop=ad)
    return K.attn_bwd(qkv, o, do, lse, geo.key_mask, B, S, nh, window, scale, geo.rope[i], geo.per_batch_pos, prescaled=True, drop=ad)


class _EncoderLayerFn(torch.autograd.Function):

    @staticmethod
    def forward(ctx, geo: _Geometry, i: int, x: Tensor, *weights: Tensor):
        it = iter(weights)
        w_an = None if i == 0 else _f32(next(it))
        Wqkv, Wo, w_mn, Wi, Wo2 = next(it), next(it), _f32(next(it)), next(it), next(it)
        fuse_geglu = (not geo.save) and not (geo.drop is not None and geo.drop.mlp) and Wi.dim() == 2 and K.gemm_geglu_supported(x.shape[0], Wi.shape[0] // 2, Wi.shape[1]) \
            and os.environ.get("CM3P_GEGLU_FUSED", "1") != "0"
        pre = geo.wcast if geo.save and geo.wcast is not None else {}
        pairs = [pre.get(id(w)) or _bf16_weight_pair(w, geo.save) if not (fuse_geglu and w is Wi) else (None, None) for w in (Wqkv, Wo, Wi, Wo2)]
        wb = (w_an, pairs[0][0], pairs[1][0], w_mn, pairs[2][0], pairs[3][0], _bf16_weight_cached(Wi, True) if fuse_geglu else None)
        x_out, acts = _layer_forward(geo, i, x, wb, geo.save)
        if geo.save:
            ctx.saved = (x,) if geo.checkpoint else acts
            ctx.geo, ctx.i, ctx.wb = geo, i, wb
            ctx.wt = tuple(p[1] for p in pairs)
            ctx.wdtypes = [w.dtype for w in weights]
        return x_out

    @staticmethod
    def _backward_bf16(ctx, dy: Tensor):
        geo, i = ctx.geo, ctx.i
        need = ctx.needs_input_grad
        need_w = list(need[3:])
        if i == 0:
            need_w.insert(0, False)
        n_an, n_qkv, n_o, n_mn, n_i, n_o2 = need_w
        g = _take_bf16_from_downstream(geo, dy)
        if geo.checkpoint:
            _, acts = _layer_forward(geo, i, ctx.saved[0], ctx.wb, True)
        else:
            acts = ctx.saved
        x, xn, mean_a, rstd_a, qkv, o, lse, x_mid, xn2, mean_m, rstd_m, h, ga = acts
        del acts
        w_an, Wqkv_b, Wo_b, w_mn, Wi_b, Wo2_b = ctx.wb[:6]
        Wqkv_t, Wo_t, Wi_t, Wo2_t = ctx.wt
        ctx.saved = ctx.wb = ctx.wt = None
        dg = K.linear_dgrad(g, Wo2_b, Wo2_t)
        dWo2 = K.linear_wgrad(g, ga) if n_o2 else None
        dh = K.geglu_bwd(dg, h)
        del dg, ga
        dxn2 = K.linear_dgrad(dh, Wi_b, Wi_t)
        dWi = K.linear_wgrad(dh, xn2) if n_i else None
        del dh, h, xn2
        _, g, dw_mn = K.layernorm_bwd(dxn2, x_mid, w_mn, mean_m, rstd_m, g, False, bf16_only=True)
        del dxn2, x_mid
        do = K.linear_dgrad(g, Wo_b, Wo_t)
        dWo = K.linear_wgrad(g, o) if n_o else None
        dqkv = _attn_backward(geo, i, qkv, o, do, lse, None)
        del do, o, qkv
        dWqkv = K.linear_wgrad(dqkv, xn) if n_qkv else None
        dw_an = None
        if i == 0:
            if need[2]:
                _, g = K.add_f32(g, K.linear_dgrad(dqkv, Wqkv_b, Wqkv_t))
            _hand_upstream(geo, g, g)
        elif need[2] or n_an:
            dxn = K.linear_dgrad(dqkv, Wqkv_b, Wqkv_t)
            _, g, dw_an = K.layernorm_bwd(dxn, x, w_an, mean_a, rstd_a, g, False, bf16_only=True)
            _hand_upstream(geo, g, g)
        grads = [dWqkv, dWo, dw_mn, dWi, dWo2] if i == 0 else [dw_an, dWqkv, dWo, dw_mn, dWi, dWo2]
        out = [(gw if gw.dtype == dt else gw.to(dt)) if (nd and gw is not None) else None for gw, dt, nd in zip(grads, ctx.wdtypes, need[3:])]
        return (None, None, g if need[2] else None, *out)

    @staticmethod
    def backward(ctx, dy: Tensor):
        if ctx.geo.bf16:
            return _EncoderLayerFn._backward_bf16(ctx, dy)
        geo, i = ctx.geo, ctx.i
        need = ctx.needs_input_grad
        need_w = list(need[3:])
        if i == 0:
            need_w.insert(0, False)
        n_an, n_qkv, n_o, n_mn, n_i, n_o2 = need_w
        gx32, gx16 = _take_from_downstream(geo, dy)
        if geo.checkpoint:
            _, acts = _layer_forward(geo, i, ctx.saved[0], ctx.wb, True)
        else:
            acts = ctx.saved
        x, xn, mean_a, rstd_a, qkv, o, lse, x_mid, xn2, mean_m, rstd_m, h, g = acts
        del acts
        w_an, Wqkv_b, Wo_b, w_mn, Wi_b, Wo2_b = ctx.wb[:6]
        Wqkv_t, Wo_t, Wi_t, Wo2_t = ctx.wt
        ctx.saved = ctx.wb = ctx.wt = None
        dg = K.linear_dgrad(gx16, Wo2_b, Wo2_t)
        dWo2 = K.linear_wgrad(gx16, g) if n_o2 else None
        if geo.drop is not None and geo.drop.mlp:
            dh = K.geglu_bwd_dropout(dg, h, geo.drop.mlp, geo.drop.seed, i, geo.S, geo.cu)
        else:
            dh = K.geglu_bwd(dg, h)
        del dg, g
        dxn2 = K.linear_dgrad(dh, Wi_b, Wi_t)
        dWi = K.linear_wgrad(dh, xn2) if n_i else None
        del dh, h, xn2
        gx32, gx16, dw_mn = K.layernorm_bwd(dxn2, x_mid, w_mn, mean_m, rstd_m, gx32, True)
        del dxn2, x_mid
        ad = (geo.drop.attn, geo.drop.seed, i) if geo.drop is not None and geo.drop.attn else None
        gt16 = gx16 if ad is None else K.dropout_f32(gx32, ad[0], ad[1], i, K.SITE_ATTN_OUT, geo.S, geo.cu, bf16_only=True)
        do = K.linear_dgrad(gt16, Wo_b, Wo_t)
        dWo = K.linear_wgrad(gt16, o) if n_o else None
        del gt16
        dqkv = _attn_backward(geo, i, qkv, o, do, lse, ad)
        del do, o, qkv
        dWqkv = K.linear_wgrad(dqkv, xn) if n_qkv else None
        if i == 0:
            dw_an = None
            if need[2]:
                dxn = K.linear_dgrad(dqkv, Wqkv_b, Wqkv_t)
                gx32, _ = K.add_f32(gx32, dxn, want_bf16=False)
            _hand_upstream(geo, gx32, None)
        elif need[2] or n_an:
            dxn = K.linear_dgrad(dqkv, Wqkv_b, Wqkv_t)
            gx32, gx16, dw_an = K.layernorm_bwd(dxn, x, w_an, mean_a, rstd_a, gx32, True)
            _hand_upstream(geo, gx32, gx16)
        else:
            dw_an = None
        grads = [dWqkv, dWo, dw_mn, dWi, dWo2] if i == 0 else [dw_an, dWqkv, dWo, dw_mn, dWi, dWo2]
        out = [(gw if gw.dtype == dt else gw.to(dt)) if (nd and gw is not None) else None for gw, dt, nd in zip(grads, ctx.wdtypes, need[3:])]
        return (None, None, gx32 if need[2] else None, *out)


class _FinalNormFn(torch.autograd.Function):

    @staticmethod
    def forward(ctx, geo: _Geometry, x: Tensor, norm_w: Tensor):
        w = _f32(norm_w.detach())
        if geo.bf16:
            _, y, mean, rstd = K.layernorm_fwd(x, w, geo.eps, False, True, geo.save)
            if geo.save:
                ctx.geo, ctx.pack, ctx.wdtype = geo, (x, w, mean, rstd), norm_w.dtype
            return y
        y, _, mean, rstd = K.layernorm_fwd(x, w, geo.eps, True, False, geo.save)
        if geo.save:
            ctx.geo, ctx.pack, ctx.wdtype = geo, (x, w, mean, rstd), norm_w.dtype
        return y

    @staticmethod
    def backward(ctx, dy: Tensor):
        x, w, mean, rstd = ctx.pack
        if ctx.geo.bf16:
            _, g, dw = K.layernorm_bwd(dy.to(torch.bfloat16).contiguous(), x, w, mean, rstd, None, False, inplace=False, bf16_only=True)
            ctx.pack = None
            _hand_upstream(ctx.geo, g, g)
            return None, g if ctx.needs_input_grad[1] else None, dw.to(ctx.wdtype) if ctx.needs_input_grad[2] else None
        gx32, gx16, dw = K.layernorm_bwd(dy.contiguous(), x, w, mean, rstd, None, True, inplace=False)
        ctx.pack = None
        _hand_upstream(ctx.geo, gx32, gx16)
        return None, gx32 if ctx.needs_input_grad[1] else None, dw.to(ctx.wdtype) if ctx.needs_input_grad[2] else None


class _EmbedLNFn(torch.autograd.Function):

    @staticmethod
    def forward(ctx, ids: Tensor, table: Tensor, norm_w: Tensor, eps: float, padding_idx: int, slot: Optional[Tensor],
                audio_rows: Optional[Tensor], bf16: bool = False):
        w = _f32(norm_w.detach())
        tab = table.detach()
        ar = audio_rows.detach().contiguous() if audio_rows is not None else None
        if bf16:
            _, y, mean, rstd = K.embed_ln_fwd(ids, tab, w, eps, slot, ar, want_bf16=True, want_f32=False)
        else:
            y, _, mean, rstd = K.embed_ln_fwd(ids, tab, w, eps, slot, ar)
        ctx.pack = (ids, tab, w, mean, rstd, slot, ar, padding_idx)
        ctx.dtypes = (table.dtype, norm_w.dtype, audio_rows.dtype if audio_rows is not None else None)
        return y

    @staticmethod
    def backward(ctx, dy: Tensor):
        ids, tab, w, mean, rstd, slot, ar, padding_idx = ctx.pack
        d_table, d_audio, dw = K.embed_ln_bwd(dy.contiguous(), ids, tab, w, mean, rstd, padding_idx, slot, ar,
# ... 196 lines not shown
        dev = ref.device

        packed = None
        if unpad and attention_mask is not None and input_ids is not None:
            packed = self._plan_unpadded(attention_mask.reshape(B, S), position_ids)

        if packed is not None:
            idx, cu, max_s, n_valid, n_rows, pos = packed
            ids = input_ids.contiguous().view(-1)[idx]
            slot_p = None
            if audio_slot is not None:
                slot_p = audio_slot.view(-1)[idx]
            if n_rows != n_valid:
                ids = torch.cat((ids, ids.new_zeros(n_rows - n_valid)))
                if slot_p is not None:
                    slot_p = torch.cat((slot_p, slot_p.new_full((n_rows - n_valid,), -1)))
            pad = self.embeddings.tok_embeddings.padding_idx
            x0 = _EmbedLNFn.apply(ids, self.embeddings.tok_embeddings.weight, self.embeddings.norm.weight, cfg.norm_eps,
                                  -1 if pad is None else pad, None if slot_p is None else slot_p.contiguous(), audio_rows, bf16)
        elif input_ids is not None:
            pad = self.embeddings.tok_embeddings.padding_idx
            x0 = _EmbedLNFn.apply(input_ids.contiguous().view(-1), self.embeddings.tok_embeddings.weight,
                                  self.embeddings.norm.weight, cfg.norm_eps, -1 if pad is None else pad, audio_slot, audio_rows, bf16)
        else:
            x0 = _LayerNormFn.apply(inputs_embeds.reshape(B * S, H), self.embeddings.norm.weight, cfg.norm_eps, bf16)

        x0 = self._embed_dropout(x0, plan, S, packed[1] if packed is not None else None)
        y, hiddens, attns = self._run_stack(x0, B, S, attention_mask, position_ids, packed, output_hidden_states, dev, output_attentions, plan, bf16)
        if hiddens is not None:
            if packed is not None:
                hiddens = [K.scatter_rows(h[:n_valid].contiguous(), idx, B * S) for h in hiddens]
            hiddens = tuple(h.view(B, S, H) for h in hiddens)
        if packed is not None:
            y = _PadRowsFn.apply(y, idx, n_valid, B * S)
        y = y.view(B, S, H)
        if output_attentions:
            return y, hiddens, attns
        return (y, hiddens) if output_hidden_states else y

    def _run_stack(self, x0: Tensor, B: int, S: int, attention_mask, position_ids, packed, output_hidden_states: bool, dev,
                   output_attentions: bool = False, plan: Optional[_DropPlan] = None, bf16: bool = False):
        cfg = self.config
        H = cfg.hidden_size
        geo = _Geometry()
        geo.B, geo.S, geo.H, geo.I, geo.nh, geo.L = B, S, H, cfg.intermediate_size, cfg.num_attention_heads, cfg.num_hidden_layers
        geo.hd = H // cfg.num_attention_heads
        geo.eps = cfg.norm_eps
        geo.windows = [-1 if cfg.is_global_layer(i) else cfg.half_window for i in range(geo.L)]
        geo.key_mask = None
        geo.cu = None
        geo.checkpoint = bool(self.gradient_checkpointing and self.training)
        geo.drop = plan
        geo.max_s = S
        if packed is not None:
            idx, cu, max_s, n_valid, n_rows, pos = packed
            geo.B = cu.numel() - 1
            geo.S = max_s
            geo.cu, geo.max_s = cu, max_s
            geo.per_batch_pos = True
            pos_tok = pos
        else:
            if attention_mask is not None:
                geo.key_mask = (attention_mask.reshape(B, S) != 0).to(torch.uint8).contiguous()
            if position_ids is None:
                position_ids = torch.arange(S, device=dev).unsqueeze(0)
            geo.per_batch_pos = position_ids.shape[0] != 1
            if geo.per_batch_pos and position_ids.shape[0] != B:
                raise ValueError("position_ids must be (1, S) or (B, S)")
            pos_tok = position_ids.contiguous().to(torch.int64)
        tables = {}
        for is_global, theta in ((True, cfg.global_rope_theta), (False, cfg.local_rope_theta)):
            if any(cfg.is_global_layer(i) == is_global for i in range(geo.L)):
                tables[is_global] = K.rope_table(pos_tok, self._inv_freq(theta, dev))
        geo.rope = [tables[cfg.is_global_layer(i)] for i in range(geo.L)]
        weights = self._stack_weights()
        geo.save = torch.is_grad_enabled() and (x0.requires_grad or self.final_norm.weight.requires_grad
                                                or any(w.requires_grad for ws in weights for w in ws))
        if bf16 and geo.save and (self._train_residual_dtype is not torch.bfloat16 or plan is not None):
            raise RuntimeError("cm3p_amd: bf16 residual stream on a call that records a backward without train_residual_dtype, or with dropout")
        geo.bf16 = bf16
        if geo.save and _eval_weights:
            invalidate_weight_cache()
        geo.wcast = None
        if geo.save and os.environ.get("CM3P_CAST_BATCHED", "1") != "0":
            elig = [w for ws in weights for w in ws
                    if w.dim() == 2 and w.dtype == torch.float32 and w.shape[0] % 8 == 0 and w.shape[1] % 8 == 0 and w.is_contiguous()]
            if elig:
                geo.wcast = {id(w): pair for w, pair in zip(elig, K.cast_bf16_with_transpose_many([w.detach() for w in elig]))}
        geo.handoff = None
        geo.attn_out = [] if output_attentions else None
        hiddens = [x0.detach()] if output_hidden_states else None
        x = x0
        for i in range(geo.L):
            x = _EncoderLayerFn.apply(geo, i, x, *weights[i])
            if hiddens is not None:
                hiddens.append(x.detach())
        y = _FinalNormFn.apply(geo, x, self.final_norm.weight)
        attns = tuple(geo.attn_out) if geo.attn_out is not None else None
        geo.attn_out = None
        return y, hiddens, attns

    def _forward_prepacked(self, input_ids: Tensor, position_ids: Optional[Tensor], audio_slot, audio_rows, cu_seqlens: Tensor,
                           max_seqlen: Optional[int], output_hidden_states: bool, plan: Optional[_DropPlan] = None, bf16: bool = False):
        cfg = self.config
        if input_ids is None or input_ids.dim() != 1:
            raise ValueError("with cu_seqlens, input_ids must be the 1-D unpadded token tensor (total_nnz,)")
        if not input_ids.is_cuda:
            raise RuntimeError("cm3p_amd runs on MI355X only: inputs must be CUDA/HIP tensors (no CPU fallback)")
        dev = input_ids.device
        ids = input_ids.to(torch.int64).contiguous()
        total = ids.numel()
        cu = cu_seqlens.to(device=dev, dtype=torch.int32).reshape(-1).contiguous()
        if cu.numel() < 2:
            raise ValueError("cu_seqlens needs at least two entries (batch + 1)")
        lens = cu[1:] - cu[:-1]
        first, last, mx, mn = torch.stack((cu[0], cu[-1], lens.max(), lens.min())).tolist()
        if first != 0 or last != total or mn <= 0:
            raise ValueError(f"cu_seqlens must start at 0, increase strictly and end at the token count ({total}); got end {last}, min length {mn}")
        max_s = int(mx) if max_seqlen is None else int(max_seqlen)
        if max_s < mx:
            raise ValueError(f"max_seqlen {max_s} is smaller than the longest sequence ({mx})")
        n_rows = (total + 63) // 64 * 64
        if position_ids is None:
            pos = torch.arange(total, device=dev) - torch.repeat_interleave(cu[:-1].to(torch.int64), lens.to(torch.int64))
        else:
            pos = position_ids.reshape(-1).to(torch.int64)
            if pos.numel() != total:
                raise ValueError("position_ids must be unpadded like input_ids")
        slot_p = audio_slot
        if n_rows != total:
            ids = torch.cat((ids, ids.new_zeros(n_rows - total)))
            pos = torch.cat((pos, torch.arange(n_rows - total, device=dev)))
            cu = torch.cat((cu, cu.new_full((1,), n_rows)))
            if slot_p is not None:
                slot_p = torch.cat((slot_p, slot_p.new_full((n_rows - total,), -1)))
        pad = self.embeddings.tok_embeddings.padding_idx
        x0 = _EmbedLNFn.apply(ids, self.embeddings.tok_embeddings.weight, self.embeddings.norm.weight, cfg.norm_eps,
                              -1 if pad is None else pad, None if slot_p is None else slot_p.contiguous(), audio_rows, bf16)
        packed = (None, cu, max(max_s, n_rows - total), total, n_rows, pos.contiguous())
        x0 = self._embed_dropout(x0, plan, max_s, cu)
        y, hiddens, _ = self._run_stack(x0, cu.numel() - 1, max_s, None, None, packed, output_hidden_states, dev, plan=plan, bf16=bf16)
        if n_rows != total:
            y = y[:total]
            if hiddens is not None:
                hiddens = [h[:total] for h in hiddens]
        return (y, tuple(hiddens)) if output_hidden_states else y

    @staticmethod
    def _plan_unpadded(mask: Tensor, position_ids: Optional[Tensor]):
        B, S = mask.shape
        m = mask != 0
        lens = m.sum(dim=1, dtype=torch.int32)
        last = (m * torch.arange(1, S + 1, device=mask.device)).amax(dim=1).to(torch.int32)
        total, max_s, min_s, prefix = torch.stack((lens.sum(), lens.max(), lens.min(), (last == lens).all().to(torch.int32))).tolist()
        if total == B * S or min_s == 0 or not prefix:
            return None
        idx = torch.nonzero(m.flatten()).flatten()
        n_rows = (total + 63) // 64 * 64
        seq = lens if n_rows == total else torch.cat((lens, lens.new_full((1,), n_rows - total)))
        cu = torch.zeros(seq.numel() + 1, dtype=torch.int32, device=mask.device)
        cu[1:] = torch.cumsum(seq, 0)
        if position_ids is None:
            pos = idx % S
        else:
            pos = position_ids.expand(B, S).reshape(-1)[idx]
        if n_rows != total:
            pos = torch.cat((pos, torch.arange(n_rows - total, device=mask.device)))
        return idx, cu, max(int(max_s), n_rows - total), int(total), int(n_rows), pos.contiguous().to(torch.int64)
```

### cm3p_amd/kernels.py

```python
from __future__ import annotations

import math
import os
from typing import Optional

import torch

from . import _lib
from ._lib import ADD_A_BF16, BF16, GEMM_F32_TILED, POOL_PACKED, EPI_BF16, EPI_BF16_RESID, EPI_F32, EPI_F32_RESID, F32, call, dt, ptr, query, stream

Tensor = torch.Tensor

_lib.HBM_BOUND_TAGS.update({"cm3p_layernorm_fwd", "cm3p_layernorm_bwd", "cm3p_geglu_fwd", "cm3p_geglu_bwd", "attn_bwd_prep_kernel [global]",
                            "attn_bwd_dq_reduce_kernel [global]", "attn_bwd_prep_kernel [global, varlen]", "attn_bwd_dq_reduce_kernel [global, varlen]"})


def _empty(shape, dtype, like: Tensor) -> Tensor:
    return torch.empty(shape, dtype=dtype, device=like.device)


def layernorm_fwd(x: Tensor, weight: Tensor, eps: float, want_f32: bool, want_bf16: bool, want_stats: bool = True):
    rows, H = x.shape
    y32 = _empty((rows, H), torch.float32, x) if want_f32 else None
    y16 = _empty((rows, H), torch.bfloat16, x) if want_bf16 else None
    mean = _empty((rows,), torch.float32, x) if want_stats else None
    rstd = _empty((rows,), torch.float32, x) if want_stats else None
    call("cm3p_layernorm_fwd", ptr(x), dt(x), ptr(weight, torch.float32), ptr(y32), ptr(y16), ptr(mean, torch.float32), ptr(rstd, torch.float32), rows, H, eps, stream(),
         work=float(rows) * H * (x.element_size() + (4 if want_f32 else 0) + (2 if want_bf16 else 0)))
    return y32, y16, mean, rstd


def layernorm_bwd(dy: Tensor, x: Tensor, weight: Tensor, mean: Tensor, rstd: Tensor, dres: Optional[Tensor],
                  want_bf16: bool, inplace: bool = True, bf16_only: bool = False):
    rows, H = x.shape
    if bf16_only:
        dx32 = None
        dx16 = dres if (inplace and dres is not None and dres.dtype == torch.bfloat16) else _empty((rows, H), torch.bfloat16, x)
    else:
        dx32 = dres if (inplace and dres is not None and dres.dtype == torch.float32) else _empty((rows, H), torch.float32, x)
        dx16 = _empty((rows, H), torch.bfloat16, x) if want_bf16 else None
    nblk = query("cm3p_layernorm_bwd_blocks", rows)
    part = _empty((nblk, H), torch.float32, x)
    dw = _empty((H,), torch.float32, x)
    call("cm3p_layernorm_bwd", ptr(dy), dt(dy), ptr(x), dt(x), ptr(weight, torch.float32), ptr(mean, torch.float32), ptr(rstd, torch.float32), ptr(dres),
         dt(dres) if dres is not None else F32, ptr(dx32), ptr(dx16), ptr(part), ptr(dw), rows, H, stream(),
         work=float(rows) * H * (dy.element_size() + x.element_size() + (dres.element_size() if dres is not None else 0)
                                 + (4 if dx32 is not None else 0) + (2 if dx16 is not None else 0)))
    return dx32, dx16, dw


def embed_ln_fwd(ids: Tensor, table: Tensor, weight: Tensor, eps: float, slot: Optional[Tensor] = None,
                 override: Optional[Tensor] = None, want_bf16: bool = False, want_f32: bool = True):
    T = ids.numel()
    H = table.shape[1]
    if not (want_f32 or want_bf16):
        raise ValueError("embed_ln_fwd: no output requested")
    y32 = _empty((T, H), torch.float32, table) if want_f32 else None
    y16 = _empty((T, H), torch.bfloat16, table) if want_bf16 else None
    mean = _empty((T,), torch.float32, table)
    rstd = _empty((T,), torch.float32, table)
    call("cm3p_embed_ln_fwd", ptr(ids, torch.int64), ptr(table), dt(table), ptr(slot, torch.int32), ptr(override), dt(override) if override is not None else F32,
         ptr(weight, torch.float32), ptr(y32), ptr(y16), ptr(mean, torch.float32), ptr(rstd, torch.float32), T, H, eps, table.shape[0], stream())
    return y32, y16, mean, rstd


def embed_ln_bwd(dy: Tensor, ids: Tensor, table: Tensor, weight: Tensor, mean: Tensor, rstd: Tensor, padding_idx: int,
                 slot: Optional[Tensor] = None, override: Optional[Tensor] = None, want_table_grad: bool = True):
    T = ids.numel()
    V, H = table.shape
    if want_table_grad and T > 0 and os.environ.get("CM3P_EMBED_BWD", "sorted") != "atomic":
        return _embed_ln_bwd_sorted(dy, ids, table, weight, mean, rstd, padding_idx, slot, override)
    d_table = torch.zeros((V, H), dtype=torch.float32, device=table.device) if want_table_grad else None
    d_ovr = torch.zeros(override.shape, dtype=torch.float32, device=table.device) if override is not None else None
    nblk = query("cm3p_layernorm_bwd_blocks", T)
    part = _empty((nblk, H), torch.float32, table)
    dw = _empty((H,), torch.float32, table)
    call("cm3p_embed_ln_bwd", ptr(dy), dt(dy), ptr(ids, torch.int64), ptr(table), dt(table), ptr(slot, torch.int32), ptr(override),
         dt(override) if override is not None else F32, ptr(weight, torch.float32), ptr(mean, torch.float32), ptr(rstd, torch.float32), ptr(d_table), ptr(d_ovr), ptr(part), ptr(dw),
         T, H, padding_idx, V, stream())
    return d_table, d_ovr, dw


def _embed_ln_bwd_sorted(dy, ids, table, weight, mean, rstd, padding_idx, slot, override):
    T = ids.numel()
    V, H = table.shape
    dev = table.device
    chunk = query("cm3p_embed_ln_bwd_sorted_chunk")
    flat = ids.reshape(-1).to(torch.int64).contiguous()
    order, run_of = token_order(flat, V, chunk)
    R = min(T, V + 3 + T // chunk)
    run_rows = _empty((R, H), torch.float32, table)
    run_ids = torch.empty((R,), dtype=torch.int64, device=dev)
# ... 42 lines not shown

_GEMM_KERNELS = ("gemm_bf16_kernel", "gemm256_kernel", "gemm8p_kernel")
_GEMM_RING, _GEMM_REBAL = 2, 4
EPI_ROPE, EPI_GEGLU = 3, 6


def _gemm_tag(M: int, N: int, K: int, a_kc, b_kc, epilogue, split_k: int, lda: Optional[int] = None, ldb: Optional[int] = None,
              rope_cols: int = 0, kernel: Optional[int] = None) -> str:
    lda = (K if a_kc else M) if lda is None else lda
    ldb = (K if b_kc else N) if ldb is None else ldb
    code = query("cm3p_gemm_route", M, N, K, lda, ldb, int(bool(a_kc)), int(bool(b_kc)), epilogue, split_k, rope_cols, 0)
    if code < 0:
        raise _lib.Cm3pHipError(f"cm3p_gemm_route: no bf16 GEMM kernel takes M {M} N {N} K {K} a_kc {a_kc} b_kc {b_kc} epilogue {epilogue} split_k {split_k}")
    kernel = code & 3 if kernel is None else kernel
    b2s = lambda v: "true" if v else "false"
    tail = f", {b2s(code & _GEMM_REBAL)}" if kernel == _GEMM_RING else ""
    return f"{_GEMM_KERNELS[kernel]}<{b2s(a_kc)}, {b2s(b_kc)}, {epilogue}{tail}>"


def gemm(a: Tensor, b: Tensor, M: int, N: int, K: int, a_kc: bool, b_kc: bool, epilogue: int,
         resid: Optional[Tensor] = None, out: Optional[Tensor] = None, split_k: int = 1) -> Tensor:
    lda, ldb = a.shape[1], b.shape[1]
    if out is None:
        out = _empty((M, N), torch.bfloat16 if epilogue in (EPI_BF16, EPI_BF16_RESID) else torch.float32, a)
    ws = _empty((split_k, M, N), torch.float32, a) if split_k > 1 else None
    call("cm3p_gemm_bf16", ptr(a), ptr(b), ptr(out), ptr(resid), M, N, K, lda, ldb, N, int(a_kc), int(b_kc), epilogue, split_k,
         ptr(ws), stream(), tag=_gemm_tag(M, N, K, a_kc, b_kc, epilogue, split_k, lda, ldb), work=2.0 * M * N * K)
    return out


def linear_fwd(x: Tensor, w: Tensor, resid: Optional[Tensor] = None) -> Tensor:
    T, K = x.shape
    N = w.shape[0]
    if resid is None:
        return gemm(x, w, T, N, K, True, True, EPI_BF16)
    return gemm(x, w, T, N, K, True, True, EPI_BF16_RESID if resid.dtype == torch.bfloat16 else EPI_F32_RESID, resid)


def linear_fwd_f32(x: Tensor, w: Tensor) -> Tensor:
    T, K = x.shape
    return gemm(x, w, T, w.shape[0], K, True, True, EPI_F32, None)


SOFTMAX_Q_SCALE = 64 ** -0.5 * 1.4426950408889634


def qkv_linear_rope(x: Tensor, w: Tensor, cos: Tensor, sin: Tensor, S: int, per_batch: bool, q_scale: float = 1.0) -> Tensor:
    T, Kd = x.shape
    N = w.shape[0]
    out = _empty((T, N), torch.bfloat16, x)
    call("cm3p_qkv_gemm_rope", ptr(x), ptr(w), ptr(out), T, N, Kd, ptr(cos, torch.float32), ptr(sin, torch.float32), S, int(per_batch), 2 * N // 3, float(q_scale), stream(),
         tag=_gemm_tag(T, N, Kd, True, True, EPI_ROPE, 1, rope_cols=2 * N // 3), work=2.0 * T * N * Kd)
    return out


def linear_dgrad(dy: Tensor, w: Tensor, w_t: Optional[Tensor] = None) -> Tensor:
    T, N = dy.shape
    K = w.shape[1]
    if w_t is not None:
        return gemm(dy, w_t, T, K, N, True, True, EPI_BF16)
    return gemm(dy, w, T, K, N, True, False, EPI_BF16)


def linear_wgrad(dy: Tensor, x: Tensor) -> Tensor:
    T, N = dy.shape
    K = x.shape[1]
    return gemm(dy, x, N, K, T, False, False, EPI_F32, split_k=_wgrad_splits(N, K, T))


def cast_bf16(x: Tensor) -> Tensor:
    y = torch.empty(x.shape, dtype=torch.bfloat16, device=x.device)
    call("cm3p_cast_f32_bf16", ptr(x, torch.float32), ptr(y), x.numel(), stream())
    return y


def cast_bf16_with_transpose(x: Tensor):
    rows, cols = x.shape
    y = torch.empty((rows, cols), dtype=torch.bfloat16, device=x.device)
    yt = torch.empty((cols, rows), dtype=torch.bfloat16, device=x.device)
    call("cm3p_cast_f32_bf16_t", ptr(x, torch.float32), ptr(y), ptr(yt), rows, cols, stream())
    return y, yt


def cast_bf16_with_transpose_many(ws: list) -> list:
    if not ws:
        return []
    dev = ws[0].device
    numel = sum(w.numel() for w in ws)
    store = torch.empty((2 * numel,), dtype=torch.bfloat16, device=dev)
    base, out, table, off, blocks = store.data_ptr(), [], [], 0, 0
    for w in ws:
        rows, cols = w.shape
        y = store[off:off + rows * cols].view(rows, cols)
        yt = store[off + rows * cols:off + 2 * rows * cols].view(cols, rows)
        table += [w.data_ptr(), base + 2 * off, base + 2 * (off + rows * cols), rows, cols, blocks]
        out.append((y, yt))
        off += 2 * rows * cols
        blocks += (-(-rows // 64)) * (-(-cols // 64))
    tab = torch.tensor(table, dtype=torch.int64).pin_memory().to(dev, non_blocking=True)
    call("cm3p_cast_f32_bf16_t_multi", ptr(tab, torch.int64), len(ws), blocks, stream(), work=8.0 * numel)
    return out


def add_f32(a: Tensor, b: Tensor, want_bf16: bool = False, inplace: bool = True):
    if a.dtype == torch.bfloat16:
        y16 = a if inplace else torch.empty_like(a)
        call("cm3p_add_f32", ptr(a), ptr(b), dt(b) | ADD_A_BF16, None, ptr(y16), a.numel(), stream())
        return None, y16
    y32 = a if inplace else torch.empty_like(a)
    y16 = torch.empty(a.shape, dtype=torch.bfloat16, device=a.device) if want_bf16 else None
    call("cm3p_add_f32", ptr(a), ptr(b), dt(b), ptr(y32), ptr(y16), a.numel(), stream())
    return y32, y16


def rope_table(position_ids: Tensor, inv_freq: Tensor):
    n = position_ids.numel()
    half = inv_freq.numel()
    cos = torch.empty((n, half), dtype=torch.float32, device=inv_freq.device)
    sin = torch.empty((n, half), dtype=torch.float32, device=inv_freq.device)
    call("cm3p_rope_table", ptr(position_ids, torch.int64), n, ptr(inv_freq, torch.float32), half, ptr(cos, torch.float32), ptr(sin, torch.float32), stream())
    return cos, sin


def rope_apply_(qkv: Tensor, cos: Tensor, sin: Tensor, B: int, S: int, nh: int, per_batch: bool, inverse: bool = False):
    call("cm3p_rope_apply", ptr(qkv), ptr(cos, torch.float32), ptr(sin, torch.float32), B, S, nh, S if per_batch else 0, int(inverse), stream())
    return qkv


def gemm8p_set_grid(workgroups: int) -> None:
    rc = _lib.load().cm3p_gemm8p_set_grid(int(workgroups))
    if rc != 0:
        raise ValueError(f"cm3p_gemm8p_set_grid({workgroups}) -> {rc}")


def gemm8p_get_grid() -> int:
    return int(_lib.load().cm3p_gemm8p_get_grid())


def _drop_abi(drop: Optional[tuple]) -> tuple:
    if drop is None:
        return "", (), ">"
    thr, seed, layer = drop
    return "_dropout", (layer, thr, seed), ", DropCfg>"


def _attn_fwd_name(window: int, prescaled: bool, masked: bool, S: int, nh: int, targs_end: str = ">") -> str:
    if targs_end == ">" and query("cm3p_attn_fwd_impl", S, nh, window, int(prescaled)):
        return "attn_fwd_g_kernel<4, " + ("true>" if masked else "false>")
    return "attn_fwd_kernel<1, %s, " + ("true" if window >= 0 else "false") + targs_end


def attn_fwd(qkv: Tensor, key_mask: Optional[Tensor], B: int, S: int, nh: int, window: int, scale: float, prescaled: bool = False,
             drop: Optional[tuple] = None):
    out = torch.empty((B * S, nh * 64), dtype=torch.bfloat16, device=qkv.device)
    lse = torch.empty((B, nh, S), dtype=torch.float32, device=qkv.device)
    keys = S if window < 0 else min(S, 2 * window + 1)
    sfx, drop_args, targs_end = _drop_abi(drop)
    call("cm3p_attn_fwd" + sfx, ptr(qkv), ptr(out), ptr(lse, torch.float32), ptr(key_mask, torch.uint8), B, S, nh, window, scale, int(prescaled),
         *drop_args, stream(), tag=_attn_tag(_attn_fwd_name(window, prescaled, key_mask is not None, S, nh, targs_end), window, prescaled),
         work=4.0 * B * nh * S * keys * 64)
    return out, lse


HD_MFMA_SIZES = (96, 128)


def attn_generic_supported(head_dim: int) -> bool:
    return bool(query("cm3p_attn_generic_supported", int(head_dim)))


def _attn_hd_prof(names: tuple, products: int, B: int, S: int, nh: int, hd: int, window: int) -> dict:
    if hd not in HD_MFMA_SIZES:
        return {}
    keys = S if window < 0 else min(S, 2 * window + 1)
    return dict(tag=_attn_tag(" + ".join(f"{n}<{hd}>" for n in names), window, False), work=2.0 * products * B * nh * S * keys * hd)


def rope_apply_generic_(qkv: Tensor, cos: Tensor, sin: Tensor, B: int, S: int, nh: int, hd: int, per_batch: bool, inverse: bool = False):
# ... 95 lines not shown
    for stage, name, products in ((ATTN_BWD_DQ, "attn_bwd_dq_kernel<%s", 1), (ATTN_BWD_DKV, "attn_bwd_dkv_kernel<%s", 3)):
        call("cm3p_attn_bwd" + sfx, ptr(qkv), ptr(out), ptr(dout), ptr(lse, torch.float32), ptr(delta), ptr(dqkv), ptr(key_mask, torch.uint8), B, S, nh,
             window, scale, ptr(cos, torch.float32), ptr(sin, torch.float32), S if per_batch else 0, stage, int(prescaled), *drop_args, stream(),
             tag=_attn_tag(name + targs_end, window, prescaled), work=None if drop is not None else 2.0 * products * B * nh * S * keys * 64)
    return dqkv


def attn_fwd_varlen(qkv: Tensor, cu: Tensor, B: int, max_s: int, nh: int, window: int, scale: float, prescaled: bool = False,
                    drop: Optional[tuple] = None):
    total = qkv.shape[0]
    out = torch.empty((total, nh * 64), dtype=torch.bfloat16, device=qkv.device)
    lse = torch.empty((nh, total), dtype=torch.float32, device=qkv.device)
    sfx, drop_args, targs_end = _drop_abi(drop)
    call("cm3p_attn_fwd" + sfx + "_varlen", ptr(qkv), ptr(out), ptr(lse, torch.float32), ptr(cu, torch.int32), B, max_s, total, nh, window, scale,
         int(prescaled), *drop_args, stream(), tag=_attn_tag(_attn_fwd_name(window, prescaled, False, max_s, nh, targs_end), window, prescaled, True))
    return out, lse


def attn_bwd_varlen(qkv: Tensor, out: Tensor, dout: Tensor, lse: Tensor, cu: Tensor, B: int, max_s: int, nh: int, window: int,
                    scale: float, rope: Optional[tuple] = None, prescaled: bool = False, drop: Optional[tuple] = None) -> Tensor:
    if drop is None and window < 0:
        return _attn_bwd_fused(qkv, out, dout, lse, None, cu, B, max_s, qkv.shape[0], nh, scale, rope, False, prescaled)
    dqkv = torch.empty_like(qkv)
    delta = torch.empty_like(lse)
    cos, sin = rope if rope is not None else (None, None)
    sfx, drop_args, targs_end = _drop_abi(drop)
    for stage, name in ((ATTN_BWD_DQ, "attn_bwd_dq_kernel<%s"), (ATTN_BWD_DKV, "attn_bwd_dkv_kernel<%s")):
        call("cm3p_attn_bwd" + sfx + "_varlen", ptr(qkv), ptr(out), ptr(dout), ptr(lse, torch.float32), ptr(delta), ptr(dqkv), ptr(cu, torch.int32), B,
             max_s, qkv.shape[0], nh, window, scale, ptr(cos, torch.float32), ptr(sin, torch.float32), stage, int(prescaled), *drop_args, stream(),
             tag=_attn_tag(name + targs_end, window, prescaled, True))
    return dqkv


def _rows_as_f32(src: Tensor) -> Tensor:
    return src.view(torch.float32) if src.dtype == torch.bfloat16 else src


def gather_rows(src: Tensor, idx: Tensor) -> Tensor:
    s32 = _rows_as_f32(src)
    out = torch.empty((idx.numel(), s32.shape[1]), dtype=torch.float32, device=src.device)
    if idx.numel() == 0:
        return out.view(src.dtype)
    call("cm3p_gather_rows_f32", ptr(s32), ptr(idx, torch.int64), ptr(out), idx.numel(), s32.shape[1], stream())
    return out.view(src.dtype)


def scatter_rows(src: Tensor, idx: Tensor, rows: int) -> Tensor:
    s32 = _rows_as_f32(src)
    out = torch.zeros((rows, s32.shape[1]), dtype=torch.float32, device=src.device)
    if idx.numel() == 0:
        return out.view(src.dtype)
    call("cm3p_scatter_rows_f32", ptr(s32), ptr(idx, torch.int64), ptr(out), idx.numel(), s32.shape[1], stream())
    return out.view(src.dtype)


def geglu_fwd(h: Tensor) -> Tensor:
    T, I2 = h.shape
    g = torch.empty((T, I2 // 2), dtype=torch.bfloat16, device=h.device)
    call("cm3p_geglu_fwd", ptr(h), ptr(g), T, I2 // 2, stream(), work=6.0 * T * (I2 // 2))
    return g


def gemm_geglu_supported(T: int, I: int, Kd: int) -> bool:
    code = query("cm3p_gemm_route", T, 2 * I, Kd, Kd, Kd, 1, 1, EPI_GEGLU, 1, 0, 0)
    return code >= 0 and (code & 3) == _GEMM_RING


def geglu_interleave_index(I: int, device) -> Tensor:
    n = torch.arange(2 * I, device=device)
    r = n % 64
    j = (n // 64) * 32 + r % 32
    return torch.where(r < 32, j, I + j)


def gemm_geglu(x: Tensor, w_interleaved: Tensor) -> Tensor:
    T, Kd = x.shape
    I = w_interleaved.shape[0] // 2
    a = _empty((T, I), torch.bfloat16, x)
    call("cm3p_gemm_geglu", ptr(x), ptr(w_interleaved), ptr(a), T, I, Kd, stream(),
         tag=_gemm_tag(T, 2 * I, Kd, True, True, EPI_GEGLU, 1, kernel=_GEMM_RING), work=2.0 * T * 2 * I * Kd)
    return a


def geglu_bwd(dg: Tensor, h: Tensor) -> Tensor:
    dh = torch.empty_like(h)
    call("cm3p_geglu_bwd", ptr(dg), ptr(h), ptr(dh), h.shape[0], h.shape[1] // 2, stream(), work=10.0 * h.shape[0] * (h.shape[1] // 2))
    return dh


SITE_EMBED, SITE_ATTN_PROBS, SITE_ATTN_OUT, SITE_MLP = 0, 1, 2, 3


def dropout_threshold(p: float) -> int:
    return int(math.floor(float(p) * 65536.0 + 0.5))


def dropout_scale(thr: int) -> float:
    return 0.0 if thr >= 65536 else float(torch.tensor(65536.0) / torch.tensor(float(65536 - thr)))


def _drop_rows(S: int, cu: Optional[Tensor]):
    return (S, None, 0) if cu is None else (S, ptr(cu, torch.int32), cu.numel() - 1)


def dropout_f32(x: Tensor, thr: int, seed: int, layer: int, site: int, S: int, cu: Optional[Tensor] = None, resid: Optional[Tensor] = None,
                bf16_only: bool = False) -> Tensor:
    rows, H = x.shape
    y = torch.empty(x.shape, dtype=torch.bfloat16 if bf16_only else torch.float32, device=x.device)
    call("cm3p_dropout_f32", ptr(x, torch.float32), ptr(resid, torch.float32), None if bf16_only else ptr(y), ptr(y) if bf16_only else None, rows, H,
         *_drop_rows(S, cu), layer, site, thr, seed, stream())
    return y


def geglu_fwd_dropout(h: Tensor, thr: int, seed: int, layer: int, S: int, cu: Optional[Tensor] = None) -> Tensor:
    T, I2 = h.shape
    g = torch.empty((T, I2 // 2), dtype=torch.bfloat16, device=h.device)
    call("cm3p_geglu_fwd_dropout", ptr(h, torch.bfloat16), ptr(g), T, I2 // 2, *_drop_rows(S, cu), layer, thr, seed, stream())
    return g


def geglu_bwd_dropout(dg: Tensor, h: Tensor, thr: int, seed: int, layer: int, S: int, cu: Optional[Tensor] = None) -> Tensor:
    dh = torch.empty_like(h)
    call("cm3p_geglu_bwd_dropout", ptr(dg, torch.bfloat16), ptr(h, torch.bfloat16), ptr(dh), h.shape[0], h.shape[1] // 2, *_drop_rows(S, cu),
         layer, thr, seed, stream())
    return dh


def dropout_keep(n2: int, n1: int, n0: int, layer: int, site: int, thr: int, seed: int, device) -> Tensor:
    keep = torch.empty((n2, n1, n0), dtype=torch.uint8, device=device)
    call("cm3p_dropout_keep", ptr(keep), n2, n1, n0, layer, site, thr, seed, stream())
    return keep


def philox4x32_10_host(ctr, key):
    import numpy as np

    c = np.ascontiguousarray(ctr, dtype=np.uint32).reshape(-1, 4)
    k = np.ascontiguousarray(key, dtype=np.uint32).reshape(-1, 2)
    if c.shape[0] != k.shape[0]:
        raise ValueError("one key per counter")
    out = np.empty_like(c)
    _lib._check(query("cm3p_philox4x32_10_host", c.ctypes.data, k.ctypes.data, out.ctypes.data, c.shape[0]), "cm3p_philox4x32_10_host")
    return out


def gelu_fwd(x: Tensor) -> Tensor:
    y = torch.empty_like(x)
    call("cm3p_gelu_fwd", ptr(x), ptr(y), x.numel(), stream())
    return y


def gelu_bwd(dy: Tensor, x: Tensor) -> Tensor:
    dx = torch.empty_like(x)
    call("cm3p_gelu_bwd", ptr(dy), ptr(x), ptr(dx), x.numel(), stream())
    return dx


def im2col_k3(x: Tensor, token_major: bool, B: int, C: int, T_in: int, stride: int):
    T_out = (T_in - 1) // stride + 1
    p = torch.empty((B * T_out, C * 3), dtype=torch.bfloat16, device=x.device)
    call("cm3p_im2col_k3", ptr(x, torch.bfloat16 if token_major else torch.float32), int(token_major), ptr(p), B, C, T_in, T_out, stride, stream())
    return p, T_out


def col2im_k3(dp: Tensor, B: int, C: int, T_in: int, T_out: int, stride: int) -> Tensor:
    dx = torch.empty((B, T_in, C), dtype=torch.bfloat16, device=dp.device)
# ... 194 lines not shown
```

### include/cm3p_hip.h

```cpp
#ifndef CM3P_HIP_H
#define CM3P_HIP_H

#include <stdint.h>

#ifdef __cplusplus
extern "C" {
#endif

#define CM3P_OK 0
#define CM3P_ERR_INVALID (-1)
#define CM3P_ERR_LAUNCH (-2)
#define CM3P_ERR_INTERNAL (-3)

#define CM3P_F32 0
#define CM3P_BF16 1

#define CM3P_ABI_VERSION 20
int cm3p_abi_version(void);

int cm3p_layernorm_fwd(const void* x, int x_dtype, const float* weight, float* y_f32, void* y_bf16, float* mean,
                       float* rstd, int64_t rows, int H, float eps, void* stream);

int cm3p_layernorm_bwd_blocks(int64_t rows);

int cm3p_layernorm_bwd(const void* dy, int dy_dtype, const void* x, int x_dtype, const float* weight, const float* mean,
                       const float* rstd, const void* dres, int dres_dtype, float* dx_f32, void* dx_bf16, float* dw_partial,
                       float* dw, int64_t rows, int H, void* stream);

int cm3p_embed_ln_fwd(const int64_t* ids, const void* table, int table_dtype, const int32_t* slot,
                      const void* override_rows, int override_dtype, const float* weight, float* y_f32, void* y_bf16,
                      float* mean, float* rstd, int64_t T, int H, float eps, int64_t vocab, void* stream);

int cm3p_embed_ln_bwd(const void* dy, int dy_dtype, const int64_t* ids, const void* table, int table_dtype, const int32_t* slot,
                      const void* override_rows, int override_dtype, const float* weight, const float* mean,
                      const float* rstd, float* d_table, float* d_override, float* dw_partial, float* dw, int64_t T, int H,
                      int64_t padding_idx, int64_t vocab, void* stream);

int cm3p_embed_ln_bwd_sorted_chunk(void);
int cm3p_embed_ln_bwd_sorted(const void* dy, int dy_dtype, const int64_t* ids, const int64_t* order, const int32_t* run_of, const void* table,
                             int table_dtype, const int32_t* slot, const void* override_rows, int override_dtype, const float* weight,
                             const float* mean, const float* rstd, float* d_table, float* d_override, float* run_rows, int64_t* run_ids,
                             float* dw_partial, float* dw, int64_t T, int H, int64_t padding_idx, int64_t vocab, void* stream);

int64_t cm3p_token_order_workspace_ints(int64_t T, int64_t vocab);
int cm3p_token_order(const int64_t* ids, int64_t T, int64_t vocab, int64_t* order, int32_t* run_of, int32_t* workspace, void* stream);

int cm3p_audio_slots(const int64_t* ids, int64_t T, int64_t audio_token_id, int32_t* slot, int32_t* count, void* stream);

#define CM3P_EPI_BF16 0
#define CM3P_EPI_F32 1
#define CM3P_EPI_F32_RESID 2
#define CM3P_EPI_F32_BIAS 5
#define CM3P_EPI_BF16_RESID 7
int cm3p_gemm_bf16(const void* A, const void* B, void* C, const float* R, int64_t M, int64_t N, int64_t K, int64_t lda,
                   int64_t ldb, int64_t ldc, int a_kc, int b_kc, int epilogue, int split_k, float* workspace, void* stream);

int cm3p_gemm8p_set_grid(int workgroups);
int cm3p_gemm8p_get_grid(void);

int cm3p_build_ablation_flags(void);

int cm3p_debug_set_dma_audit(void* buf);

int cm3p_qkv_gemm_rope(const void* x, const void* Wqkv, void* qkv, int64_t M, int64_t N, int64_t K, const float* cos_tab,
                       const float* sin_tab, int S, int per_batch, int rope_cols, float q_scale, void* stream);

int cm3p_gemm_wgrad_splits(int64_t M, int64_t N, int64_t K);

int cm3p_gemm_route(int64_t M, int64_t N, int64_t K, int64_t lda, int64_t ldb, int a_kc, int b_kc, int epilogue, int split_k,
                    int rope_cols, int batch);

int cm3p_cast_f32_bf16(const float* x, void* y, int64_t n, void* stream);
int cm3p_cast_f32_bf16_t(const float* x, void* y, void* y_t, int64_t rows, int64_t cols, void* stream);
int cm3p_cast_f32_bf16_t_multi(const int64_t* table, int n, int64_t total_blocks, void* stream);
#define CM3P_ADD_A_BF16 16
int cm3p_add_f32(const void* a, const void* b, int b_dtype, float* y_f32, void* y_bf16, int64_t n, void* stream);

int cm3p_rope_table(const int64_t* position_ids, int64_t n_pos, const float* inv_freq, int half_dim, float* cos_out,
                    float* sin_out, void* stream);
int cm3p_rope_apply(void* qkv, const float* cos_tab, const float* sin_tab, int B, int S, int nh, int64_t pos_batch_stride,
                    int inverse, void* stream);

int cm3p_attn_fwd(const void* qkv, void* out, float* lse, const uint8_t* key_mask, int B, int S, int nh, int window,
                  float scale, int q_prescaled, void* stream);
int cm3p_attn_fwd_impl(int S, int nh, int window, int q_prescaled);

int cm3p_attn_probs(const void* qkv, const float* lse, const uint8_t* key_mask, float* probs, int B, int S, int nh, int window, float scale,
                    int q_prescaled, void* stream);
#define CM3P_ATTN_BWD_DQ 1
#define CM3P_ATTN_BWD_DKV 2
int cm3p_attn_bwd(const void* qkv, const void* out, const void* dout, const float* lse, float* delta, void* dqkv,
                  const uint8_t* key_mask, int B, int S, int nh, int window, float scale, const float* cos_tab,
                  const float* sin_tab, int64_t pos_batch_stride, int stages, int q_prescaled, void* stream);

int cm3p_attn_generic_supported(int head_dim);
int cm3p_attn_fwd_generic(const void* qkv, void* out, float* lse, const uint8_t* key_mask, int B, int S, int nh, int head_dim, int window,
                          float scale, void* stream);
int cm3p_attn_bwd_generic(const void* qkv, const void* out, const void* dout, const float* lse, float* delta, void* dqkv,
                          const uint8_t* key_mask, int B, int S, int nh, int head_dim, int window, float scale, void* stream);
int cm3p_attn_fwd_generic_dropout(const void* qkv, void* out, float* lse, const uint8_t* key_mask, int B, int S, int nh, int head_dim,
                                  int window, float scale, int layer, int thr, uint64_t seed, void* stream);
int cm3p_attn_bwd_generic_dropout(const void* qkv, const void* out, const void* dout, const float* lse, float* delta, void* dqkv,
                                  const uint8_t* key_mask, int B, int S, int nh, int head_dim, int window, float scale, int layer, int thr,
                                  uint64_t seed, void* stream);
int cm3p_rope_apply_generic(void* qkv, const float* cos_tab, const float* sin_tab, int B, int S, int nh, int head_dim, int64_t pos_batch_stride,
                            int inverse, void* stream);

#define CM3P_ATTN_BWD_FUSED_PREP 1
#define CM3P_ATTN_BWD_FUSED_MAIN 2
#define CM3P_ATTN_BWD_FUSED_REDUCE 4
#define CM3P_ATTN_BWD_FUSED_MAIN_EVEN 8
#define CM3P_ATTN_BWD_FUSED_MAIN_ODD 16
#define CM3P_ATTN_BWD_FUSED_MAIN_ADD1 32
int64_t cm3p_attn_bwd_fused_workspace_bytes(int B, int S, int nh);
int cm3p_attn_bwd_fused_slab_group(int S);
int cm3p_attn_bwd_fused(const void* qkv, const void* out, const void* dout, const float* lse, void* dqkv, const uint8_t* key_mask,
                        const int* cu_seqlens, int B, int S, int64_t total, int nh, float scale, const float* cos_tab,
                        const float* sin_tab, int64_t pos_batch_stride, int stages, int q_prescaled, void* workspace,
                        int64_t workspace_bytes, void* stream);

int cm3p_attn_fwd_dropout(const void* qkv, void* out, float* lse, const uint8_t* key_mask, int B, int S, int nh, int window, float scale,
                          int q_prescaled, int layer, int thr, uint64_t seed, void* stream);
int cm3p_attn_bwd_dropout(const void* qkv, const void* out, const void* dout, const float* lse, float* delta, void* dqkv,
                          const uint8_t* key_mask, int B, int S, int nh, int window, float scale, const float* cos_tab,
                          const float* sin_tab, int64_t pos_batch_stride, int stages, int q_prescaled, int layer, int thr, uint64_t seed,
                          void* stream);
int cm3p_attn_fwd_dropout_varlen(const void* qkv, void* out, float* lse, const int* cu_seqlens, int B, int max_seqlen, int64_t total, int nh,
                                 int window, float scale, int q_prescaled, int layer, int thr, uint64_t seed, void* stream);
int cm3p_attn_bwd_dropout_varlen(const void* qkv, const void* out, const void* dout, const float* lse, float* delta, void* dqkv,
                                 const int* cu_seqlens, int B, int max_seqlen, int64_t total, int nh, int window, float scale,
                                 const float* cos_tab, const float* sin_tab, int stages, int q_prescaled, int layer, int thr, uint64_t seed,
                                 void* stream);

int cm3p_geglu_fwd(const void* h, void* g, int64_t T, int I, void* stream);

int cm3p_gemm_geglu(const void* x, const void* w_interleaved, void* a, int64_t T, int64_t I, int64_t K, void* stream);
// ... 83 lines not shown
```

Measured before the change: 198.0 pairs/s.

## Fuse GeGLU activation into MLP up-projection and down-projection dgrad GEMM epilogues

Adds two GEMM epilogues on the ring kernel. The forward up-projection writes both the pre-activation h and the GeGLU output. The backward Wo2 dgrad computes the GeGLU backward directly from the accumulators and writes dh. To make the gate and up columns land in the same tile, the training weight cast stores Wi rows interleaved in 32-row chunks. This removes the separate geglu and geglu_bwd elementwise passes and their extra HBM round trips of the T×I tensors. The cost is heavier epilogues and a different weight layout for the fused path.

```diff
diff --git a/cm3p_amd/_lib.py b/cm3p_amd/_lib.py
--- a/cm3p_amd/_lib.py
+++ b/cm3p_amd/_lib.py
@@ -11,6 +11,7 @@
 POOL_PACKED = 2
 GEMM_F32_TILED = 2
 EPI_BF16, EPI_F32, EPI_F32_RESID, EPI_F32_BIAS, EPI_BF16_RESID = 0, 1, 2, 5, 7
+EPI_BF16_GEGLU_FWD, EPI_BF16_GEGLU_BWD = 9, 10
 ABI_VERSION = 20
 
 _HERE = os.path.dirname(os.path.abspath(__file__))
diff --git a/cm3p_amd/csrc/common.h b/cm3p_amd/csrc/common.h
--- a/cm3p_amd/csrc/common.h
+++ b/cm3p_amd/csrc/common.h
@@ -25,6 +25,7 @@
     int64_t a_stride = 0, b_stride = 0, c_stride = 0, r_stride = 0;
     const uint16_t* Rb = nullptr;
     float alpha = 1.f, beta = 0.f;
+    void* C2 = nullptr;
 };
 
 #ifndef CM3P_NT
@@ -206,6 +207,32 @@
 __device__ __forceinline__ float bf16hi(uint32_t w) { return __builtin_bit_cast(float, w & 0xffff0000u); }
 __device__ __forceinline__ uint32_t add_bf16x2(uint32_t a, uint32_t b) { return pack_bf16x2(bf16lo(a) + bf16lo(b), bf16hi(a) + bf16hi(b)); }
 
+__device__ __forceinline__ void unpack8(const uint4 w, float (&f)[8]) {
+    f[0] = bf16lo(w.x); f[1] = bf16hi(w.x); f[2] = bf16lo(w.y); f[3] = bf16hi(w.y);
+    f[4] = bf16lo(w.z); f[5] = bf16hi(w.z); f[6] = bf16lo(w.w); f[7] = bf16hi(w.w);
+}
+__device__ __forceinline__ uint4 pack8(const float (&f)[8]) {
+    return uint4{pack_bf16x2(f[0], f[1]), pack_bf16x2(f[2], f[3]), pack_bf16x2(f[4], f[5]), pack_bf16x2(f[6], f[7])};
+}
+__device__ __forceinline__ void geglu_bwd_item_f(const uint4 ha, const uint4 hb, const float (&d)[8], uint4& oa, uint4& ob) {
+    float a[8], b[8], da[8], db[8];
+    unpack8(ha, a);
+    unpack8(hb, b);
+#pragma unroll
+    for (int j = 0; j < 8; j += 2) {
+        const f32x2 av = {a[j], a[j + 1]};
+        f32x2 cdf, pdf;
+        gelu_cdf_pdf2(av, cdf, pdf);
+        const f32x2 gr = av * pdf + cdf, gl = av * cdf;
+        da[j] = d[j] * b[j] * gr.x;
+        da[j + 1] = d[j + 1] * b[j + 1] * gr.y;
+        db[j] = d[j] * gl.x;
+        db[j + 1] = d[j + 1] * gl.y;
+    }
+    oa = pack8(da);
+    ob = pack8(db);
+}
+
 struct RopeArgs {
     const float* cos;
     const float* sin;
@@ -254,11 +281,16 @@
         case CM3P_EPI_F32_BIAS: return f(std::integral_constant<int, CM3P_EPI_F32_BIAS>{});
         case CM3P_EPI_BF16_GEGLU: return f(std::integral_constant<int, CM3P_EPI_BF16_GEGLU>{});
         case CM3P_EPI_BF16_RESID: return f(std::integral_constant<int, CM3P_EPI_BF16_RESID>{});
+        case CM3P_EPI_BF16_GEGLU_FWD: return f(std::integral_constant<int, CM3P_EPI_BF16_GEGLU_FWD>{});
+        case CM3P_EPI_BF16_GEGLU_BWD: return f(std::integral_constant<int, CM3P_EPI_BF16_GEGLU_BWD>{});
         default: return CM3P_ERR_INTERNAL;
     }
 }
+constexpr bool cm3p_epi_is_geglu(int epi) {
+    return epi == CM3P_EPI_BF16_GEGLU || epi == CM3P_EPI_BF16_GEGLU_FWD || epi == CM3P_EPI_BF16_GEGLU_BWD;
+}
 constexpr bool cm3p_gemm_pair_exists(bool a_kc, bool b_kc, int epi) {
-    return (epi != CM3P_EPI_BF16_ROPE && epi != CM3P_EPI_F32_BIAS && epi != CM3P_EPI_BF16_GEGLU) || (a_kc && b_kc);
+    return (epi != CM3P_EPI_BF16_ROPE && epi != CM3P_EPI_F32_BIAS && !cm3p_epi_is_geglu(epi)) || (a_kc && b_kc);
 }
 
 template <bool INVERSE>
diff --git a/cm3p_amd/csrc/elementwise.hip b/cm3p_amd/csrc/elementwise.hip
--- a/cm3p_amd/csrc/elementwise.hip
+++ b/cm3p_amd/csrc/elementwise.hip
@@ -10,13 +10,6 @@
     return (int)blocks;
 }
 
-__device__ __forceinline__ void unpack8(const uint4 w, float (&f)[8]) {
-    f[0] = bf16lo(w.x); f[1] = bf16hi(w.x); f[2] = bf16lo(w.y); f[3] = bf16hi(w.y);
-    f[4] = bf16lo(w.z); f[5] = bf16hi(w.z); f[6] = bf16lo(w.w); f[7] = bf16hi(w.w);
-}
-__device__ __forceinline__ uint4 pack8(const float (&f)[8]) {
-    return uint4{pack_bf16x2(f[0], f[1]), pack_bf16x2(f[2], f[3]), pack_bf16x2(f[4], f[5]), pack_bf16x2(f[6], f[7])};
-}
 
 __global__ __launch_bounds__(256) void cast_f32_bf16_kernel(const float* __restrict__ x, uint16_t* __restrict__ y, int64_t n4) {
     for (int64_t i = (int64_t)blockIdx.x * 256 + threadIdx.x; i < n4; i += (int64_t)gridDim.x * 256) {
@@ -67,7 +60,9 @@
     const float* x = reinterpret_cast<const float*>(table[6 * lo]);
     uint16_t* y = reinterpret_cast<uint16_t*>(table[6 * lo + 1]);
     uint16_t* yt = reinterpret_cast<uint16_t*>(table[6 * lo + 2]);
-    const int rows = (int)table[6 * lo + 3], cols = (int)table[6 * lo + 4];
+    const int rows_arg = (int)table[6 * lo + 3], cols = (int)table[6 * lo + 4];
+    const bool interleave = rows_arg < 0;
+    const int rows = interleave ? -rows_arg : rows_arg, half = rows >> 1;
     const int blk = (int)((int64_t)blockIdx.x - table[6 * lo + 5]);
     const int tiles_c = (cols + 63) / 64;
     const int r0 = (blk / tiles_c) * 64, c0 = (blk % tiles_c) * 64;
@@ -78,7 +73,9 @@
         if (r0 + r < rows && c0 + c < cols) {
             const f32x4 v = *reinterpret_cast<const f32x4*>(x + (int64_t)(r0 + r) * cols + c0 + c);
             const uint32_t lo2 = pack_bf16x2(v.x, v.y), hi2 = pack_bf16x2(v.z, v.w);
-            *reinterpret_cast<uint2*>(y + (int64_t)(r0 + r) * cols + c0 + c) = uint2{lo2, hi2};
+            int yr = r0 + r;
+            if (interleave) yr = yr < half ? (yr >> 5) * 64 + (yr & 31) : ((yr - half) >> 5) * 64 + 32 + ((yr - half) & 31);
+            *reinterpret_cast<uint2*>(y + (int64_t)yr * cols + c0 + c) = uint2{lo2, hi2};
             tile[r][c] = (uint16_t)lo2;
             tile[r][c + 1] = (uint16_t)(lo2 >> 16);
             tile[r][c + 2] = (uint16_t)hi2;
@@ -248,25 +245,6 @@
     }
 }
 
-__device__ __forceinline__ void geglu_bwd_item_f(const uint4 ha, const uint4 hb, const float (&d)[8], uint4& oa, uint4& ob) {
-    float a[8], b[8], da[8], db[8];
-    unpack8(ha, a);
-    unpack8(hb, b);
-#pragma unroll
-    for (int j = 0; j < 8; j += 2) {
-        const f32x2 av = {a[j], a[j + 1]};
-        f32x2 cdf, pdf;
-        gelu_cdf_pdf2(av, cdf, pdf);
-        const f32x2 gr = av * pdf + cdf, gl = av * cdf;
-        da[j] = d[j] * b[j] * gr.x;
-        da[j + 1] = d[j + 1] * b[j + 1] * gr.y;
-        db[j] = d[j] * gl.x;
-        db[j + 1] = d[j + 1] * gl.y;
-    }
-    oa = pack8(da);
-    ob = pack8(db);
-}
-
 __device__ __forceinline__ void geglu_bwd_item(const uint4 ha, const uint4 hb, const uint4 hd, uint4& oa, uint4& ob) {
     float d[8];
     unpack8(hd, d);
diff --git a/cm3p_amd/csrc/gemm.hip b/cm3p_amd/csrc/gemm.hip
--- a/cm3p_amd/csrc/gemm.hip
+++ b/cm3p_amd/csrc/gemm.hip
@@ -196,7 +196,7 @@
 }
 
 template <bool A_KC, bool B_KC, int EPI>
-constexpr bool has_instance = cm3p_gemm_pair_exists(A_KC, B_KC, EPI) && EPI != CM3P_EPI_BF16_GEGLU;
+constexpr bool has_instance = cm3p_gemm_pair_exists(A_KC, B_KC, EPI) && !cm3p_epi_is_geglu(EPI);
 
 int launch128(const GemmRoute& r, const GemmCall& g, hipStream_t s) {
     const int tiles_m = (int)((g.M + BM - 1) / BM), tiles_n = (int)((g.N + BN - 1) / BN);
@@ -231,7 +231,7 @@
                                     int split_k, int rope_cols, int batch) {
     GemmRoute r{CM3P_GEMM_128, false, 1, K};
     const bool batched = epi == CM3P_EPI_BF16_AXPBY;
-    if (M <= 0 || N <= 0 || K <= 0 || split_k < 1 || epi < 0 || epi > CM3P_EPI_BF16_RESID || batched != (batch > 0) ||
+    if (M <= 0 || N <= 0 || K <= 0 || split_k < 1 || epi < 0 || epi > CM3P_EPI_BF16_GEGLU_BWD || epi == 8  || batched != (batch > 0) ||
         !cm3p_gemm_pair_exists(a_kc, b_kc, epi)) {
         r.kernel = CM3P_ERR_INVALID;
         return r;
@@ -250,6 +250,9 @@
     if (epi == CM3P_EPI_BF16_GEGLU) {
         if (!(big && N % 64 == 0 && ring_ok)) r.kernel = CM3P_ERR_INVALID;
         else r.kernel = no_ring ? CM3P_GEMM_256 : CM3P_GEMM_RING;
+    } else if (epi == CM3P_EPI_BF16_GEGLU_FWD || epi == CM3P_EPI_BF16_GEGLU_BWD) {
+        const int64_t cols = epi == CM3P_EPI_BF16_GEGLU_FWD ? 64 : 32;
+        r.kernel = (big && N % cols == 0 && ring_ok && split_k == 1 && !no_ring && !small_only) ? CM3P_GEMM_RING : CM3P_ERR_INVALID;
     } else if (batched) {
         const bool filled = M * N * batch * 10 >= items * 65536 * 7;
         big = big && filled && (a_kc || !b_kc) && ring_ok && !no_ring;
@@ -349,19 +352,24 @@
 int cm3p_gemm_bf16(const void* A, const void* B, void* C, const float* R, int64_t M, int64_t N, int64_t K, int64_t lda,
                    int64_t ldb, int64_t ldc, int a_kc, int b_kc, int epilogue, int split_k, float* workspace, void* stream) {
     CM3P_REQUIRE(A && B && C && M > 0 && N > 0 && K > 0);
-    CM3P_REQUIRE((epilogue >= CM3P_EPI_BF16 && epilogue <= CM3P_EPI_F32_RESID) || epilogue == CM3P_EPI_F32_BIAS || epilogue == CM3P_EPI_BF16_RESID);
+    const bool geglu_fwd = epilogue == CM3P_EPI_BF16_GEGLU_FWD, geglu_bwd = epilogue == CM3P_EPI_BF16_GEGLU_BWD;
+    CM3P_REQUIRE((epilogue >= CM3P_EPI_BF16 && epilogue <= CM3P_EPI_F32_RESID) || epilogue == CM3P_EPI_F32_BIAS || epilogue == CM3P_EPI_BF16_RESID ||
+                 geglu_fwd || geglu_bwd);
     CM3P_REQUIRE(cm3p_aligned16(A) && cm3p_aligned16(B) && cm3p_aligned16(C));
     CM3P_REQUIRE(lda % 8 == 0 && ldb % 8 == 0 && ldc % 4 == 0 && N % 4 == 0);
     CM3P_REQUIRE(a_kc ? (K % 8 == 0 && lda >= K) : (M % 8 == 0 && lda >= M));
     CM3P_REQUIRE(b_kc ? (K % 8 == 0 && ldb >= K) : (N % 8 == 0 && ldb >= N));
     CM3P_REQUIRE(ldc >= N);
-    CM3P_REQUIRE((epilogue != CM3P_EPI_F32_RESID && epilogue != CM3P_EPI_F32_BIAS && epilogue != CM3P_EPI_BF16_RESID) || (R && cm3p_aligned16(R)));
+    CM3P_REQUIRE((epilogue != CM3P_EPI_F32_RESID && epilogue != CM3P_EPI_F32_BIAS && epilogue != CM3P_EPI_BF16_RESID && !geglu_bwd) || (R && cm3p_aligned16(R)));
+    CM3P_REQUIRE(!geglu_fwd || (workspace && cm3p_aligned16(workspace) && ldc == N && N % 64 == 0 && split_k == 1));
+    CM3P_REQUIRE(!geglu_bwd || (ldc == 2 * N && N % 32 == 0 && split_k == 1));
     CM3P_REQUIRE(epilogue != CM3P_EPI_BF16_RESID || (N % 8 == 0 && ldc % 8 == 0));
     CM3P_REQUIRE(split_k >= 1 && (split_k == 1 || (epilogue == CM3P_EPI_F32 && workspace && cm3p_aligned16(workspace) && ldc == N)));
     const GemmRoute r = cm3p_gemm_route_of(M, N, K, lda, ldb, a_kc != 0, b_kc != 0, epilogue, split_k, 0, 0);
     CM3P_REQUIRE(r.kernel >= 0);
     hipStream_t s = static_cast<hipStream_t>(stream);
     GemmCall g{A, B, C, R, M, N, K, lda, ldb, ldc, a_kc != 0, b_kc != 0, epilogue};
+    if (geglu_fwd) g.bt.C2 = workspace;
     if (r.splits > 1) {
         g.C = workspace;
         g.c_split_stride = M * N;
diff --git a/cm3p_amd/csrc/gemm256.hip b/cm3p_amd/csrc/gemm256.hip
--- a/cm3p_amd/csrc/gemm256.hip
+++ b/cm3p_amd/csrc/gemm256.hip
@@ -356,7 +356,7 @@
 }
 
 template <bool A_KC, bool B_KC, int EPI>
-constexpr bool has_instance = cm3p_gemm_pair_exists(A_KC, B_KC, EPI) && EPI != CM3P_EPI_BF16_GEGLU && EPI != CM3P_EPI_BF16_AXPBY;
+constexpr bool has_instance = cm3p_gemm_pair_exists(A_KC, B_KC, EPI) && !cm3p_epi_is_geglu(EPI) && EPI != CM3P_EPI_BF16_AXPBY;
 
 }
 
diff --git a/cm3p_amd/csrc/gemm8p.hip b/cm3p_amd/csrc/gemm8p.hip
--- a/cm3p_amd/csrc/gemm8p.hip
+++ b/cm3p_amd/csrc/gemm8p.hip
@@ -412,6 +412,96 @@
                     G8P_GLOBAL(gstore16<(CM3P_NT & 1) != 0>(Cb + (uint32_t)(i4 * 16 + row) * ldcb + dc * 16, y));
                 if constexpr (CM3P_G8P_ABL & 1) asm volatile("" ::"v"(y));
             }
+        } else if constexpr (EPI == CM3P_EPI_BF16_GEGLU_FWD) {
+            char* Cb = reinterpret_cast<char*>(static_cast<uint16_t*>(Cv) + mw * ldc + nw);
+            char* Ab = reinterpret_cast<char*>(static_cast<uint16_t*>(bt.C2) + mw * (ldc / 2) + nw / 2);
+            const uint32_t ldcb = (uint32_t)ldc * 2, ldab = (uint32_t)ldc;
+#pragma unroll
+            for (int i4 = 0; i4 < 8; ++i4) {
+                char* eb = ebuf + (i4 & 1) * 2048;
+#pragma unroll
+                for (int j4 = 0; j4 < 4; ++j4) {
+                    const f32x4 a = acc[i4][j4];
+                    const int row = lane & 15, s8 = (j4 * 4 + (lane >> 4)) ^ ((row & 7) << 1);
+                    *reinterpret_cast<uint2*>(eb + row * 128 + s8 * 8) = uint2{pack_bf16x2(a.x, a.y), pack_bf16x2(a.z, a.w)};
+                }
+                G8P_LANE_XCHG_FENCE();
+                const int r0 = lane >> 3, r1 = 8 + (lane >> 3), ch = lane & 7;
+                const int row = lane >> 2, dc = lane & 3;
+                const u32x4 x0 = *reinterpret_cast<const u32x4*>(eb + r0 * 128 + ((ch ^ (r0 & 7)) << 4));
+                const u32x4 x1 = *reinterpret_cast<const u32x4*>(eb + r1 * 128 + ((ch ^ (r1 & 7)) << 4));
+                const u32x4 xh = *reinterpret_cast<const u32x4*>(eb + row * 128 + ((dc ^ (row & 7)) << 4));
+                const u32x4 xg = *reinterpret_cast<const u32x4*>(eb + row * 128 + (((dc + 4) ^ (row & 7)) << 4));
+                G8P_LANE_XCHG_FENCE();
+                const bool col_ok = FULL || nw + ch * 8 < N;
+                if (FULL || (col_ok && mw + i4 * 16 + r0 < M)) G8P_GLOBAL(gstore16<(CM3P_NT & 1) != 0>(Cb + (uint32_t)(i4 * 16 + r0) * ldcb + ch * 16, x0));
+                if (FULL || (col_ok && mw + i4 * 16 + r1 < M)) G8P_GLOBAL(gstore16<(CM3P_NT & 1) != 0>(Cb + (uint32_t)(i4 * 16 + r1) * ldcb + ch * 16, x1));
+                u32x4 y;
+#pragma unroll
+                for (int t = 0; t < 4; ++t) {
+                    const f32x2 gl = gelu_erf2(f32x2{bf16lo(xh[t]), bf16hi(xh[t])});
+                    y[t] = pack_bf16x2(gl.x * bf16lo(xg[t]), gl.y * bf16hi(xg[t]));
+                }
+                if (FULL || (mw + i4 * 16 + row < M && nw + dc * 8 < N))
+                    G8P_GLOBAL(gstore16<(CM3P_NT & 1) != 0>(Ab + (uint32_t)(i4 * 16 + row) * ldab + dc * 16, y));
+                if constexpr (CM3P_G8P_ABL & 1) asm volatile("" ::"v"(x0), "v"(x1), "v"(y));
+            }
+        } else if constexpr (EPI == CM3P_EPI_BF16_GEGLU_BWD) {
+            char* Cb = reinterpret_cast<char*>(static_cast<uint16_t*>(Cv) + mw * ldc + nw);
+            const char* Hb = reinterpret_cast<const char*>(reinterpret_cast<const uint16_t*>(R) + mw * ldc + 2 * nw);
+            const uint32_t ldcb = (uint32_t)ldc * 2, upb = (uint32_t)N * 2;
+            const int r0 = lane >> 3, ch = lane & 7;
+            const uint32_t hoff = (uint32_t)((ch >> 2) * 128 + (ch & 3) * 16);
+            const bool col_ok = FULL || nw + ch * 8 < N;
+            u32x4 ga0, up0, ga1, up1;
+            auto load_h = [&](int i4) {
+                const bool ok0 = FULL || (col_ok && mw + i4 * 16 + r0 < M), ok1 = FULL || (col_ok && mw + i4 * 16 + 8 + r0 < M);
+                const char* p0 = Hb + (uint32_t)(i4 * 16 + r0) * ldcb + hoff;
+                const char* p1 = Hb + (uint32_t)(i4 * 16 + 8 + r0) * ldcb + hoff;
+                const u32x4 zero = {0u, 0u, 0u, 0u};
+                if constexpr (CM3P_G8P_ABL & 1) {
+                    asm volatile("" : "=v"(ga0), "=v"(up0), "=v"(ga1), "=v"(up1) : "v"(p0), "v"(p1));
+                } else {
+                    ga0 = ok0 ? __builtin_bit_cast(u32x4, gload16<(CM3P_NT & 64) != 0>(p0)) : zero;
+                    up0 = ok0 ? __builtin_bit_cast(u32x4, gload16<(CM3P_NT & 64) != 0>(p0 + 64)) : zero;
+                    ga1 = ok1 ? __builtin_bit_cast(u32x4, gload16<(CM3P_NT & 64) != 0>(p1)) : zero;
+                    up1 = ok1 ? __builtin_bit_cast(u32x4, gload16<(CM3P_NT & 64) != 0>(p1 + 64)) : zero;
+                }
+            };
+            load_h(0);
+#pragma unroll
+            for (int i4 = 0; i4 < 8; ++i4) {
+                char* eb = ebuf + (i4 & 1) * 2048;
+#pragma unroll
+                for (int j4 = 0; j4 < 4; ++j4) {
+                    const f32x4 a = acc[i4][j4];
+                    const int row = lane & 15, s8 = (j4 * 4 + (lane >> 4)) ^ ((row & 7) << 1);
+                    *reinterpret_cast<uint2*>(eb + row * 128 + s8 * 8) = uint2{pack_bf16x2(a.x, a.y), pack_bf16x2(a.z, a.w)};
+                }
+                G8P_LANE_XCHG_FENCE();
+                const int r1 = 8 + r0;
+                const u32x4 x0 = *reinterpret_cast<const u32x4*>(eb + r0 * 128 + ((ch ^ (r0 & 7)) << 4));
+                const u32x4 x1 = *reinterpret_cast<const u32x4*>(eb + r1 * 128 + ((ch ^ (r1 & 7)) << 4));
+                G8P_LANE_XCHG_FENCE();
+                const u32x4 g0 = ga0, u0 = up0, g1 = ga1, u1 = up1;
+                if (i4 < 7) load_h(i4 + 1);
+                float d[8];
+                uint4 oa, ob;
+                unpack8(uint4{x0[0], x0[1], x0[2], x0[3]}, d);
+                geglu_bwd_item_f(uint4{g0[0], g0[1], g0[2], g0[3]}, uint4{u0[0], u0[1], u0[2], u0[3]}, d, oa, ob);
+                if (FULL || (col_ok && mw + i4 * 16 + r0 < M)) {
+                    G8P_GLOBAL(gstore16<(CM3P_NT & 1) != 0>(Cb + (uint32_t)(i4 * 16 + r0) * ldcb + ch * 16, oa));
+                    G8P_GLOBAL(gstore16<(CM3P_NT & 1) != 0>(Cb + (uint32_t)(i4 * 16 + r0) * ldcb + upb + ch * 16, ob));
+                }
+                if constexpr (CM3P_G8P_ABL & 1) asm volatile("" ::"v"(oa.x), "v"(ob.x));
+                unpack8(uint4{x1[0], x1[1], x1[2], x1[3]}, d);
+                geglu_bwd_item_f(uint4{g1[0], g1[1], g1[2], g1[3]}, uint4{u1[0], u1[1], u1[2], u1[3]}, d, oa, ob);
+                if (FULL || (col_ok && mw + i4 * 16 + r1 < M)) {
+                    G8P_GLOBAL(gstore16<(CM3P_NT & 1) != 0>(Cb + (uint32_t)(i4 * 16 + r1) * ldcb + ch * 16, oa));
+                    G8P_GLOBAL(gstore16<(CM3P_NT & 1) != 0>(Cb + (uint32_t)(i4 * 16 + r1) * ldcb + upb + ch * 16, ob));
+                }
+                if constexpr (CM3P_G8P_ABL & 1) asm volatile("" ::"v"(oa.x), "v"(ob.x));
+            }
         } else if constexpr (EPI == CM3P_EPI_BF16_AXPBY) {
             char* Cb = reinterpret_cast<char*>(static_cast<uint16_t*>(Cv) + (int64_t)z * bt.c_stride + mw * ldc + nw);
             const char* Rb = reinterpret_cast<const char*>(bt.Rb + (int64_t)z * bt.r_stride + mw * ldc + nw);
diff --git a/cm3p_amd/encoder.py b/cm3p_amd/encoder.py
--- a/cm3p_amd/encoder.py
+++ b/cm3p_amd/encoder.py
@@ -111,7 +111,7 @@
 class _Geometry:
 
     __slots__ = ("B", "S", "H", "I", "nh", "L", "eps", "windows", "key_mask", "rope", "per_batch_pos", "save", "cu", "max_s", "checkpoint",
-                 "handoff", "attn_out", "wcast", "hd", "drop", "bf16")
+                 "handoff", "attn_out", "wcast", "hd", "drop", "bf16", "fused_mlp")
 
 
 def _hand_upstream(geo: _Geometry, gx32: Tensor, gx16: Optional[Tensor]) -> None:
@@ -168,6 +168,8 @@
     _, xn2, mean_m, rstd_m = K.layernorm_fwd(x_mid, w_mn, geo.eps, False, True, want_stats)
     if len(wb) > 6 and wb[6] is not None:
         h, g = None, K.gemm_geglu(xn2, wb[6])
+    elif len(wb) > 7 and wb[7]:
+        h, g = K.linear_geglu_fwd(xn2, Wi_b)
     else:
         h = K.linear_fwd(xn2, Wi_b)
         if geo.drop is not None and geo.drop.mlp:
@@ -199,7 +201,8 @@
             and os.environ.get("CM3P_GEGLU_FUSED", "1") != "0"
         pre = geo.wcast if geo.save and geo.wcast is not None else {}
         pairs = [pre.get(id(w)) or _bf16_weight_pair(w, geo.save) if not (fuse_geglu and w is Wi) else (None, None) for w in (Wqkv, Wo, Wi, Wo2)]
-        wb = (w_an, pairs[0][0], pairs[1][0], w_mn, pairs[2][0], pairs[3][0], _bf16_weight_cached(Wi, True) if fuse_geglu else None)
+        fused_train = geo.save and id(Wi) in geo.fused_mlp
+        wb = (w_an, pairs[0][0], pairs[1][0], w_mn, pairs[2][0], pairs[3][0], _bf16_weight_cached(Wi, True) if fuse_geglu else None, fused_train)
         x_out, acts = _layer_forward(geo, i, x, wb, geo.save)
         if geo.save:
             ctx.saved = (x,) if geo.checkpoint else acts
@@ -223,12 +226,14 @@
             acts = ctx.saved
         x, xn, mean_a, rstd_a, qkv, o, lse, x_mid, xn2, mean_m, rstd_m, h, ga = acts
         del acts
-        w_an, Wqkv_b, Wo_b, w_mn, Wi_b, Wo2_b = ctx.wb[:6]
+        ctx_wb = ctx.wb
+        w_an, Wqkv_b, Wo_b, w_mn, Wi_b, Wo2_b = ctx_wb[:6]
         Wqkv_t, Wo_t, Wi_t, Wo2_t = ctx.wt
         ctx.saved = ctx.wb = ctx.wt = None
-        dg = K.linear_dgrad(g, Wo2_b, Wo2_t)
+        fused = len(ctx_wb) > 7 and ctx_wb[7]
+        dg = None if fused else K.linear_dgrad(g, Wo2_b, Wo2_t)
         dWo2 = K.linear_wgrad(g, ga) if n_o2 else None
-        dh = K.geglu_bwd(dg, h)
+        dh = K.linear_dgrad_geglu_bwd(g, Wo2_t, h) if fused else K.geglu_bwd(dg, h)
         del dg, ga
         dxn2 = K.linear_dgrad(dh, Wi_b, Wi_t)
         dWi = K.linear_wgrad(dh, xn2) if n_i else None
@@ -270,12 +275,16 @@
             acts = ctx.saved
         x, xn, mean_a, rstd_a, qkv, o, lse, x_mid, xn2, mean_m, rstd_m, h, g = acts
         del acts
-        w_an, Wqkv_b, Wo_b, w_mn, Wi_b, Wo2_b = ctx.wb[:6]
+        ctx_wb = ctx.wb
+        w_an, Wqkv_b, Wo_b, w_mn, Wi_b, Wo2_b = ctx_wb[:6]
         Wqkv_t, Wo_t, Wi_t, Wo2_t = ctx.wt
         ctx.saved = ctx.wb = ctx.wt = None
-        dg = K.linear_dgrad(gx16, Wo2_b, Wo2_t)
+        fused = len(ctx_wb) > 7 and ctx_wb[7]
+        dg = None if fused else K.linear_dgrad(gx16, Wo2_b, Wo2_t)
         dWo2 = K.linear_wgrad(gx16, g) if n_o2 else None
-        if geo.drop is not None and geo.drop.mlp:
+        if fused:
+            dh = K.linear_dgrad_geglu_bwd(gx16, Wo2_t, h)
+        elif geo.drop is not None and geo.drop.mlp:
             dh = K.geglu_bwd_dropout(dg, h, geo.drop.mlp, geo.drop.seed, i, geo.S, geo.cu)
         else:
             dh = K.geglu_bwd(dg, h)
@@ -638,11 +647,17 @@
         if geo.save and _eval_weights:
             invalidate_weight_cache()
         geo.wcast = None
+        geo.fused_mlp = frozenset()
         if geo.save and os.environ.get("CM3P_CAST_BATCHED", "1") != "0":
             elig = [w for ws in weights for w in ws
                     if w.dim() == 2 and w.dtype == torch.float32 and w.shape[0] % 8 == 0 and w.shape[1] % 8 == 0 and w.is_contiguous()]
             if elig:
-                geo.wcast = {id(w): pair for w, pair in zip(elig, K.cast_bf16_with_transpose_many([w.detach() for w in elig]))}
+                if not (plan is not None and plan.mlp) and os.environ.get("CM3P_GEGLU_FUSED", "1") != "0" \
+                        and K.mlp_geglu_fused_supported(x0.shape[0], cfg.intermediate_size, H):
+                    cast = {id(w) for w in elig}
+                    geo.fused_mlp = frozenset(id(ws[-2]) for ws in weights if id(ws[-2]) in cast and id(ws[-1]) in cast)
+                pairs = K.cast_bf16_with_transpose_many([w.detach() for w in elig], [id(w) in geo.fused_mlp for w in elig])
+                geo.wcast = {id(w): pair for w, pair in zip(elig, pairs)}
         geo.handoff = None
         geo.attn_out = [] if output_attentions else None
         hiddens = [x0.detach()] if output_hidden_states else None
diff --git a/cm3p_amd/kernels.py b/cm3p_amd/kernels.py
--- a/cm3p_amd/kernels.py
+++ b/cm3p_amd/kernels.py
@@ -7,7 +7,7 @@
 import torch
 
 from . import _lib
-from ._lib import ADD_A_BF16, BF16, GEMM_F32_TILED, POOL_PACKED, EPI_BF16, EPI_BF16_RESID, EPI_F32, EPI_F32_RESID, F32, call, dt, ptr, query, stream
+from ._lib import ADD_A_BF16, BF16, GEMM_F32_TILED, POOL_PACKED, EPI_BF16, EPI_BF16_GEGLU_BWD, EPI_BF16_GEGLU_FWD, EPI_BF16_RESID, EPI_F32, EPI_F32_RESID, F32, call, dt, ptr, query, stream
 
 Tensor = torch.Tensor
 
@@ -216,18 +216,21 @@
     return y, yt
 
 
-def cast_bf16_with_transpose_many(ws: list) -> list:
+def cast_bf16_with_transpose_many(ws: list, geglu_rows: Optional[list] = None) -> list:
     if not ws:
         return []
+    geglu_rows = geglu_rows or [False] * len(ws)
     dev = ws[0].device
     numel = sum(w.numel() for w in ws)
     store = torch.empty((2 * numel,), dtype=torch.bfloat16, device=dev)
     base, out, table, off, blocks = store.data_ptr(), [], [], 0, 0
-    for w in ws:
+    for w, il in zip(ws, geglu_rows):
         rows, cols = w.shape
+        if il and rows % 64:
+            raise ValueError(f"cast_bf16_with_transpose_many: interleaved GeGLU rows need 2I a multiple of 64, got {rows}")
         y = store[off:off + rows * cols].view(rows, cols)
         yt = store[off + rows * cols:off + 2 * rows * cols].view(cols, rows)
-        table += [w.data_ptr(), base + 2 * off, base + 2 * (off + rows * cols), rows, cols, blocks]
+        table += [w.data_ptr(), base + 2 * off, base + 2 * (off + rows * cols), -rows if il else rows, cols, blocks]
         out.append((y, yt))
         off += 2 * rows * cols
         blocks += (-(-rows // 64)) * (-(-cols // 64))
@@ -489,6 +492,31 @@
     return a
 
 
+def mlp_geglu_fused_supported(T: int, I: int, H: int) -> bool:
+    fwd = query("cm3p_gemm_route", T, 2 * I, H, H, H, 1, 1, EPI_BF16_GEGLU_FWD, 1, 0, 0)
+    bwd = query("cm3p_gemm_route", T, I, H, H, H, 1, 1, EPI_BF16_GEGLU_BWD, 1, 0, 0)
+    return fwd >= 0 and (fwd & 3) == _GEMM_RING and bwd >= 0 and (bwd & 3) == _GEMM_RING
+
+
+def linear_geglu_fwd(x: Tensor, w_interleaved: Tensor):
+    T, Kd = x.shape
+    N = w_interleaved.shape[0]
+    h = _empty((T, N), torch.bfloat16, x)
+    a = _empty((T, N // 2), torch.bfloat16, x)
+    call("cm3p_gemm_bf16", ptr(x), ptr(w_interleaved), ptr(h), None, T, N, Kd, Kd, Kd, N, 1, 1, EPI_BF16_GEGLU_FWD, 1, ptr(a), stream(),
+         tag=_gemm_tag(T, N, Kd, True, True, EPI_BF16_GEGLU_FWD, 1), work=2.0 * T * N * Kd)
+    return h, a
+
+
+def linear_dgrad_geglu_bwd(dy: Tensor, w_t: Tensor, h_interleaved: Tensor) -> Tensor:
+    T, Kd = dy.shape
+    I = w_t.shape[0]
+    dh = torch.empty_like(h_interleaved)
+    call("cm3p_gemm_bf16", ptr(dy), ptr(w_t), ptr(dh), ptr(h_interleaved), T, I, Kd, Kd, Kd, 2 * I, 1, 1, EPI_BF16_GEGLU_BWD, 1, None, stream(),
+         tag=_gemm_tag(T, I, Kd, True, True, EPI_BF16_GEGLU_BWD, 1), work=2.0 * T * I * Kd)
+    return dh
+
+
 def geglu_bwd(dg: Tensor, h: Tensor) -> Tensor:
     dh = torch.empty_like(h)
     call("cm3p_geglu_bwd", ptr(dg), ptr(h), ptr(dh), h.shape[0], h.shape[1] // 2, stream(), work=10.0 * h.shape[0] * (h.shape[1] // 2))
diff --git a/include/cm3p_hip.h b/include/cm3p_hip.h
--- a/include/cm3p_hip.h
+++ b/include/cm3p_hip.h
@@ -52,6 +52,8 @@
 #define CM3P_EPI_F32_RESID 2
 #define CM3P_EPI_F32_BIAS 5
 #define CM3P_EPI_BF16_RESID 7
+#define CM3P_EPI_BF16_GEGLU_FWD 9
+#define CM3P_EPI_BF16_GEGLU_BWD 10
 int cm3p_gemm_bf16(const void* A, const void* B, void* C, const float* R, int64_t M, int64_t N, int64_t K, int64_t lda,
                    int64_t ldb, int64_t ldc, int a_kc, int b_kc, int epilogue, int split_k, float* workspace, void* stream);
 
```

Result: faster. 200.9 pairs/s, median of 6 (+1.4%).
